# Maxwell-Zhao/RoboSimGS

Hardware: AMD Instinct MI355X
Metric: frames/sec + ms/frame (fwd, fwd+bwd) at 1M Gaussians 1920x1080 (higher is better)
Workload: dtype f32

## Files before the change

### include/mgs.h

```cpp
#ifndef MGS_H_
#define MGS_H_

#include <stddef.h>
#include <stdint.h>

#ifdef __cplusplus
extern "C" {
#endif

#define MGS_VERSION 450

#define MGS_OK 0
#define MGS_ERR_INVALID_ARGUMENT (-1)
#define MGS_ERR_WORKSPACE_TOO_SMALL (-2)
#define MGS_ERR_UNSUPPORTED (-3)

#define MGS_STATUS_ISECT_OVERFLOW 1u

#define MGS_RASTER_EXPECTED_LAST 1
#define MGS_RASTER_LATENCY 2

#define MGS_FRAMES_CLASSIC_BOUNDS 4

#define MGS_FRAMES_RADIUS_OPACITY_AWARE 8
#define MGS_FRAMES_CAMERA_ORTHO 16
#define MGS_FRAMES_CAMERA_FISHEYE 32

#define MGS_CAMERA_PINHOLE 0
#define MGS_CAMERA_ORTHO 1
#define MGS_CAMERA_FISHEYE 2

#ifndef MGS_RADIUS_CLASSIC
#define MGS_RADIUS_CLASSIC 0
#define MGS_RADIUS_OPACITY_AWARE 1
#endif
#define MGS_BIN_TIGHT 1
#define MGS_BIN_RADIUS_OPACITY_AWARE 2
#define MGS_BIN_CAMERA_ORTHO 4
#define MGS_BIN_CAMERA_FISHEYE 8

#define MGS_PARAMS_RAW 64
#define MGS_PARAMS_OPAC_PLAIN 128

#define MGS_RASTER_BWD_SPLAT_SLOTS 2
#define MGS_RASTER_BWD_RECORDS_ONLY 1

#define MGS_TILE_SIZE 16
#define MGS_MAX_CHANNELS 32

typedef void *mgs_stream_t;

int mgs_version(void);
const char *mgs_last_error_string(void);
#ifdef MGS_DEBUG_HOOKS
void mgs_debug_set_raster_cull(int enabled);
void mgs_debug_set_raster_opts(int opts);
void mgs_debug_set_sort_opts(int opts);
#endif

int mgs_projection_fwd(int n, const float *means, const float *quats, const float *scales,
                       const float *viewmat, const float *K, int width, int height,
                       float eps2d, float near_plane, float far_plane, float radius_clip,
                       int32_t *radii, float *means2d, float *depths, float *conics,
                       float *compensations, const float *opacities, int radius_rule,
                       int32_t *radii_y, int camera_model, mgs_stream_t stream);

int mgs_projection_bwd(int n, const float *means, const float *quats, const float *scales,
                       const float *viewmat, const float *K, int width, int height,
                       float eps2d, const int32_t *radii, const float *conics,
                       const float *compensations, const float *v_means2d,
                       const float *v_depths, const float *v_conics,
                       const float *v_compensations, float *v_means, float *v_quats,
                       float *v_scales, float *v_viewmat, int camera_model, mgs_stream_t stream);

int mgs_sh_fwd(int n, int degree, int coeff_stride, const float *dirs, const float *coeffs,
               const uint8_t *masks, float *colors, mgs_stream_t stream);
int mgs_sh_bwd(int n, int degree, int coeff_stride, const float *dirs, const float *coeffs,
               const uint8_t *masks, const float *v_colors, float *v_coeffs, float *v_dirs,
               mgs_stream_t stream);

int mgs_project_color_fwd(int n, const float *means, const float *quats, const float *scales,
                          const float *opacities, int sh_degree, int coeff_stride,
                          const float *sh_coeffs, const float *viewmat, const float *K,
                          int width, int height, float eps2d, float near_plane,
                          float far_plane, float radius_clip, int32_t *radii, float *means2d,
                          float *depths, float *conics, float *opac_out, int feat_stride,
                          float *feats, float *splats, int bin_flags, uint32_t *bin_info,
                          uint32_t *bin_sums, int32_t *radii_y, mgs_stream_t stream);

int mgs_isect_tiles(int n, const float *means2d, const int32_t *radii, const int32_t *radii_y, const float *depths,
                    const float *conics, const float *opacities, int tile_size, int tile_w,
                    int tile_h, int cam_id, int n_cams,
                    uint32_t isect_capacity, int32_t *tiles_per_gauss, uint32_t *n_isect,
                    uint32_t *tile_ids, int32_t *flatten_ids, int64_t *isect_ids,
                    int32_t *tile_offsets, int32_t *pair_info, int32_t *tile_group_order,
                    uint32_t *status, const uint32_t *seed_info, uint32_t *seed_sums, float *splat_slots,
                    void *workspace, size_t *workspace_bytes, mgs_stream_t stream);

int mgs_render_frames(int n, const float *means, const float *quats, const float *scales,
                      const float *opacities, int sh_degree, int coeff_stride, const float *sh_coeffs,
                      int n_cams, const float *viewmats, const float *Ks, int width, int height,
                      float eps2d, float near_plane, float far_plane, float radius_clip,
                      int antialiased, int channels, int flags, const float *backgrounds,
                      uint32_t isect_capacity, float *render, float *alphas, uint32_t *n_isect,
                      uint32_t *status, uint8_t *ds_rgba, void *ds_distance, int ds_distance_type,
                      const double *ds_Kinv_host, void *workspace, size_t *workspace_bytes, mgs_stream_t stream);

#define MGS_TRAIN_FIELDS 17
int mgs_train_state_layout(int n, int width, int height, int channels, uint32_t isect_capacity, int antialiased,
                           int checkpoint_interval, size_t *offsets, size_t *bytes_per_camera);
int mgs_render_frames_train(int n, const float *means, const float *quats, const float *scales,
                            const float *opacities, int sh_degree, int coeff_stride, const float *sh_coeffs,
                            int n_cams, const float *viewmats, const float *Ks, int width, int height,
                            float eps2d, float near_plane, float far_plane, float radius_clip, int antialiased,
                            int channels, int flags, const float *backgrounds, uint32_t isect_capacity,
                            int checkpoint_interval, float *render, float *alphas, void *state, void *workspace,
                            size_t *workspace_bytes, mgs_stream_t stream);
int mgs_render_frames_backward(int n, const float *means, const float *quats, const float *scales,
                               const float *opacities, int sh_degree, int coeff_stride, const float *sh_coeffs,
                               int n_cams, const float *viewmats, const float *Ks, int width, int height,
                               float eps2d, int antialiased, int channels, int flags, const float *backgrounds,
                               uint32_t isect_capacity, int checkpoint_interval, const float *render,
                               const float *alphas, const float *v_render, const float *v_alphas,
                               const void *state, float *v_means, float *v_quats, float *v_scales,
                               float *v_sh_coeffs, float *v_opacities, float *v_viewmats, float *v_means2d,
                               float *v_means2d_abs, void *workspace, size_t *workspace_bytes,
                               mgs_stream_t stream);

int mgs_isect_offset_encode(uint32_t n_isect, const int64_t *isect_ids, int n_cams,
                            int tile_w, int tile_h, int32_t *offsets, mgs_stream_t stream);

int mgs_rasterize_fwd(int n, const float *means2d, const float *conics, const float *feats,
                      const float *opacities, const float *splats, const float *background,
                      int channels, int width, int height, int tile_w, int tile_h,
                      const int32_t *tile_offsets, const int32_t *flatten_ids,
                      const int32_t *tile_group_order, int flags,
                      float *render, float *alphas, int32_t *last_ids, float *checkpoints,
                      int checkpoint_interval, uint8_t *ds_rgba, void *ds_distance, int ds_distance_type,
                      const double *ds_Kinv_host, mgs_stream_t stream);
size_t mgs_raster_checkpoint_floats(uint32_t isect_capacity, int tile_w, int tile_h, int channels,
                                    int checkpoint_interval);

int mgs_rasterize_bwd(int n, const float *means2d, const float *conics, const float *feats,
                      const float *opacities, const float *background, int channels,
                      int width, int height, int tile_w, int tile_h,
                      const int32_t *tile_offsets, const int32_t *flatten_ids,
                      const float *alphas, const int32_t *last_ids, const float *v_render,
                      const float *v_alphas, float *v_means2d, float *v_means2d_abs,
                      float *v_conics, float *v_feats, float *v_opacities,
                      mgs_stream_t stream);

int mgs_rasterize_bwd_det(int n, const float *means2d, const float *conics, const float *feats,
                          const float *opacities, const float *splats, const float *background,
                          int channels, int width, int height, int tile_w, int tile_h,
                          const int32_t *tile_offsets, const int32_t *flatten_ids,
                          const float *alphas, const int32_t *last_ids, const float *v_render,
                          const float *v_alphas, const float *expected_render,
                          const int32_t *pair_info, const int32_t *tile_group_order,
                          uint32_t isect_capacity, const float *render_out, const float *checkpoints,
                          int checkpoint_interval, int flags, float *v_means2d, float *v_means2d_abs,
                          float *v_conics, float *v_feats, float *v_opacities, void *workspace,
                          size_t *workspace_bytes, mgs_stream_t stream);

int mgs_project_color_bwd(int n, const float *means, const float *quats, const float *scales,
                          const float *opacities, int sh_degree, int coeff_stride,
                          const float *sh_coeffs, const float *viewmat, const float *K,
                          int width, int height, float eps2d, const int32_t *radii,
                          const float *conics, int antialiased, int feat_stride,
                          const float *feats, const float *v_feats, const float *v_means2d,
                          const float *v_conics, const float *v_depths,
                          const float *v_opac_out, float *v_means, float *v_quats,
                          float *v_scales, float *v_sh_coeffs, float *v_opacities,
                          float *v_viewmat, int accumulate, int camera_model, mgs_stream_t stream);

int mgs_composite_over(int n_px, const float *bg_rgb, const float *bg_alpha,
                       const float *bg_depth, const float *fg_rgb, const float *fg_depth,
                       const uint8_t *fg_mask, const float *backdrop, float *out_rgb,
                       float *out_depth, mgs_stream_t stream);

int mgs_frame_to_u8(int n_px, const float *rgb, int rgb_stride, const float *alpha,
                    const float *background, uint8_t *out, mgs_stream_t stream);

int mgs_frame_to_dataset(int width, int height, const float *colors, int color_stride,
                         const float *alpha, const float *background, const double *Kinv_host,
                         uint8_t *rgba, void *distance, int distance_f64, mgs_stream_t stream);

int mgs_points_project(int n, const float *pts, const float *K, const float *c2w, float *uv,
                       float *pnt_cam, mgs_stream_t stream);
int mgs_points_depth_map(int n, const float *uv, int uv_stride, const float *depth, int height,
                         int width, int cells_h, int cells_w, float scale, float bg_depth,
                         float *depth_map, int64_t *index, void *workspace,
                         size_t *workspace_bytes, mgs_stream_t stream);
int mgs_points_sample_mask(int n, const float *uv, int uv_stride, const float *mask, int height,
                           int width, float thresh, const float *depth_map,
                           const float *pnt_depth, float depth_thresh, uint8_t *out,
                           mgs_stream_t stream);

#define MGS_SSIM_VALID 0
#define MGS_SSIM_SAME 1

typedef struct mgs_image_loss {
  int images, height, width, channels;
  float ssim_weight;
  int padding;
} mgs_image_loss;

int mgs_l1_loss_fwd(size_t n, const float *a, const float *b, float *loss, void *workspace,
                    size_t *workspace_bytes, mgs_stream_t stream, const mgs_image_loss *image);
int mgs_l1_loss_bwd(size_t n, const float *a, const float *b, const float *v_loss, float *v_a,
                    mgs_stream_t stream, const mgs_image_loss *image);
int mgs_l1_loss_fwd_grad(size_t n, const float *a, const float *b, float *loss, float *v_a,
                         void *workspace, size_t *workspace_bytes, mgs_stream_t stream,
                         const mgs_image_loss *image);
int mgs_l1_loss_bwd_scale(size_t n, const float *v_loss, float *v_a, mgs_stream_t stream);

int mgs_transform_gaussians(int n, const float *means, const float *quats, const float *scales,
                            int sh_degree, int coeff_stride, const float *sh_coeffs,
                            const int32_t *group_ids, int n_groups, const float *xforms,
                            const float *sh_rot, float *out_means, float *out_quats,
                            float *out_scales, float *out_sh, mgs_stream_t stream);

#ifdef __cplusplus
}
#endif
#endif
```

### robosimgs_amd/csrc/binning.hip

```cpp
#include "mgs_common.h"
#include "tile_rect.h"
#include "tile_order.h"

namespace mgs {
namespace {

constexpr int kBlock = 128;

__device__ __forceinline__ uint32_t wave_sum(uint32_t v) {
#pragma unroll
  for (int d = 32; d >= 1; d >>= 1) v += __shfl_xor(v, d);
  return v;
}

constexpr int kSum = 64;
__global__ __launch_bounds__(kBlock) void tile_count_kernel(
    int n, const float* __restrict__ means2d, const int32_t* __restrict__ radii,
    const int32_t* __restrict__ radii_y, const float* __restrict__ conics, const float* __restrict__ opacities,
    float tile_size, int tile_w, int tile_h, uint2* __restrict__ ginfo, uint32_t* __restrict__ sums) {
  int g = blockIdx.x * kBlock + threadIdx.x;
  int radius = g < n ? radii[g] : 0;
  uint2 info = make_uint2(kEmptyTileRect, 0u);
  if (radius > 0) {
    float2 m = reinterpret_cast<const float2*>(means2d)[g];
    TileRect r = tile_rect(m.x, m.y, radius, radii_y ? radii_y[g] : radius, tile_size, tile_w, tile_h);
    if (conics)
      r = tighten_rect(r, m.x, m.y, conics[3 * (size_t)g], conics[3 * (size_t)g + 1],
                       conics[3 * (size_t)g + 2], opacities[g], tile_size);
    info = pack_tile_rect(r);
  }
  if (g < n) ginfo[g] = info;
  const uint32_t c = wave_sum(info.y);
  const int first = blockIdx.x * kBlock + (int)(threadIdx.x & ~63u);
  if ((threadIdx.x & 63) == 0 && first < n) sums[first / kSum] = c;
}

constexpr int kScanThreads = 1024;
constexpr int kScanPerThread = 16;
template <int kScanThreads>
__device__ __forceinline__ void scan_blocksums_body(
    uint32_t nblk, uint32_t* __restrict__ blocksums, uint32_t capacity,
    uint32_t* __restrict__ n_isect, uint32_t* __restrict__ status) {
  __shared__ uint32_t ws[kScanThreads / 64];
  const unsigned lane = threadIdx.x & 63, wave = threadIdx.x >> 6;
  uint32_t running = 0;
  bool wrapped = false;
  for (uint32_t b0 = 0; b0 < nblk; b0 += kScanThreads * kScanPerThread) {
    const uint32_t b = b0 + threadIdx.x * kScanPerThread;
    uint32_t v[kScanPerThread], sum = 0;
    if (b + kScanPerThread <= nblk) {
      const uint4* src = reinterpret_cast<const uint4*>(blocksums + b);
      const uint4 q0 = src[0], q1 = src[1], q2 = src[2], q3 = src[3];
      v[0] = q0.x; v[1] = q0.y; v[2] = q0.z; v[3] = q0.w; v[4] = q1.x; v[5] = q1.y; v[6] = q1.z; v[7] = q1.w;
      v[8] = q2.x; v[9] = q2.y; v[10] = q2.z; v[11] = q2.w; v[12] = q3.x; v[13] = q3.y; v[14] = q3.z; v[15] = q3.w;
    } else {
#pragma unroll
      for (int j = 0; j < kScanPerThread; ++j) v[j] = b + j < nblk ? blocksums[b + j] : 0u;
    }
#pragma unroll
    for (int j = 0; j < kScanPerThread; ++j) sum += v[j];
    uint32_t incl = sum;
#pragma unroll
    for (int d = 1; d < 64; d <<= 1) {
      uint32_t t = __shfl_up(incl, d);
      if (lane >= (unsigned)d) incl += t;
    }
    if (lane == 63) ws[wave] = incl;
    __syncthreads();
    uint32_t off = 0, tot = 0;
    for (int w = 0; w < kScanThreads / 64; ++w) {
      if ((unsigned)w < wave) off += ws[w];
      tot += ws[w];
    }
    __syncthreads();
    uint32_t ex = running + off + incl - sum;
    uint32_t o[kScanPerThread];
#pragma unroll
    for (int j = 0; j < kScanPerThread; ++j) { o[j] = ex; ex += v[j]; }
    if (b + kScanPerThread <= nblk) {
      uint4* dst = reinterpret_cast<uint4*>(blocksums + b);
      dst[0] = make_uint4(o[0], o[1], o[2], o[3]);
      dst[1] = make_uint4(o[4], o[5], o[6], o[7]);
      dst[2] = make_uint4(o[8], o[9], o[10], o[11]);
      dst[3] = make_uint4(o[12], o[13], o[14], o[15]);
    } else {
#pragma unroll
      for (int j = 0; j < kScanPerThread; ++j)
        if (b + j < nblk) blocksums[b + j] = o[j];
    }
    wrapped |= running + tot < running;
    running += tot;
  }
  if (threadIdx.x == 0 && n_isect) {
    *n_isect = wrapped ? 0xffffffffu : running;
    *status = (wrapped || running > capacity) ? MGS_STATUS_ISECT_OVERFLOW : 0u;
  }
}
__global__ __launch_bounds__(kScanThreads) void scan_blocksums_kernel(
    uint32_t nblk, uint32_t* __restrict__ blocksums, uint32_t capacity,
    uint32_t* __restrict__ n_isect, uint32_t* __restrict__ status) {
  scan_blocksums_body<kScanThreads>(nblk, blocksums, capacity, n_isect, status);
}

__device__ __forceinline__ void store_splat_slots(float* __restrict__ splat_slots, int g, uint32_t slot_base, uint32_t rect) {
  if (splat_slots)
    *reinterpret_cast<uint2*>(splat_slots + 12 * (size_t)g + 10) = make_uint2(slot_base, rect & 0x3fffffffu);
}

__global__ __launch_bounds__(kBlock) void pair_info_kernel(
    int n, const uint2* __restrict__ ginfo, int tile_h, const uint32_t* __restrict__ blockbase,
    int4* __restrict__ pair_info, float* __restrict__ splat_slots) {
  __shared__ uint32_t ws[kBlock / 64];
  const unsigned lane = threadIdx.x & 63, wave = threadIdx.x >> 6;
  int g = blockIdx.x * kBlock + threadIdx.x;
  uint2 info = g < n ? ginfo[g] : make_uint2(1u << 20, 0u);
  uint32_t cnt = info.y;
  uint32_t incl = cnt;
#pragma unroll
  for (int d = 1; d < 64; d <<= 1) {
    uint32_t t = __shfl_up(incl, d);
    if (lane >= (unsigned)d) incl += t;
  }
  if (lane == 63) ws[wave] = incl;
  __syncthreads();
  uint32_t off = 0;
  for (int w = 0; w < kBlock / 64; ++w)
    if ((unsigned)w < wave) off += ws[w];
  if (g < n) {
    const uint32_t w = info.x >> 20;
    const uint32_t slot_base = blockbase[blockIdx.x * (kBlock / kSum)] + off + incl - cnt;
    pair_info[g] = cnt ? make_int4((int)slot_base, (int)(info.x & 1023u),
                                   (int)((info.x >> 10) & 1023u), (int)(w | ((cnt / w) << 16)))
                       : make_int4(0, 0, 0, 0);
    if (cnt) store_splat_slots(splat_slots, g, slot_base, info.x);
  }
}

__global__ __launch_bounds__(kBlock) void emit_kernel(
    int n, const uint2* __restrict__ ginfo, int tile_w, const uint32_t* __restrict__ blockbase,
    uint32_t capacity, uint32_t* __restrict__ tile_out, uint32_t* __restrict__ id_out,
    int32_t* __restrict__ tiles_per_gauss) {
  __shared__ uint32_t prefix[kBlock + 1];
  __shared__ uint32_t gid[kBlock];
  __shared__ uint32_t rpack[kBlock];
  __shared__ uint32_t ws[kBlock / 64];
  const unsigned lane = threadIdx.x & 63, wave = threadIdx.x >> 6;
  int r = blockIdx.x * kBlock + threadIdx.x;
  uint32_t cnt = 0, g = (uint32_t)r, pack = 1u << 20;
  if (r < n) {
    uint2 info = ginfo[r];
    pack = info.x;
    cnt = info.y;
    if (tiles_per_gauss) tiles_per_gauss[r] = (int32_t)cnt;
  }
  uint32_t incl = cnt;
#pragma unroll
  for (int d = 1; d < 64; d <<= 1) {
    uint32_t t = __shfl_up(incl, d);
    if (lane >= (unsigned)d) incl += t;
  }
  if (lane == 63) ws[wave] = incl;
  __syncthreads();
  uint32_t off = 0, total = 0;
  for (int w = 0; w < kBlock / 64; ++w) {
    if ((unsigned)w < wave) off += ws[w];
    total += ws[w];
  }
  prefix[threadIdx.x] = off + incl - cnt;
  if (threadIdx.x == 0) prefix[kBlock] = total;
  gid[threadIdx.x] = g;
  rpack[threadIdx.x] = pack;
  __syncthreads();
  const uint32_t base = blockbase[blockIdx.x * (kBlock / kSum)];
  for (uint32_t k0 = threadIdx.x * 4u; k0 < total; k0 += kBlock * 4u) {
    int lo = 0, hi = kBlock;
    while (hi - lo > 1) {
      int mid = (lo + hi) >> 1;
      if (prefix[mid] <= k0) lo = mid; else hi = mid;
    }
    uint32_t next = prefix[lo + 1];
    uint32_t tiles4[4], ids4[4];
#pragma unroll
    for (int i = 0; i < 4; ++i) {
      uint32_t k = k0 + i;
      while (k >= next && lo < kBlock - 1) next = prefix[++lo + 1];
      uint32_t local = k - prefix[lo];
      uint32_t p = rpack[lo];
      uint32_t w = p >> 20;
      uint32_t dy = local / w;
      uint32_t dx = local - dy * w;
      tiles4[i] = (((p >> 10) & 1023u) + dy) * (uint32_t)tile_w + (p & 1023u) + dx;
      ids4[i] = gid[lo];
    }
#pragma unroll
    for (int i = 0; i < 4; ++i) {
      uint32_t out = base + k0 + i;
      if (k0 + i < total && out < capacity) {
        tile_out[out] = tiles4[i];
        id_out[out] = ids4[i];
      }
    }
  }
}


constexpr int kDirectThreads = 512;
constexpr int kDealRun = 256;
static_assert(kDealRun % 64 == 0 && kDirectThreads % kDealRun == 0 && kDirectThreads >= kDealRun,
              "kDirectThreads must be a multiple of kDealRun, and the run a multiple of the wave");
constexpr int kDirectPerThread = 4;
constexpr int kDirectMaxBlocks = 1024;
constexpr int kDirectMaxTiles = 15000;
constexpr int kGroupShift = 2;
constexpr uint32_t kCoopRect = 24;
constexpr uint32_t kRunRect = 128;

template <class F>
__device__ __forceinline__ void for_each_tile(uint32_t pack, uint32_t cnt, uint32_t g, int tile_w, F f) {
  const bool big = cnt > kCoopRect;
  if (!big) {
    const uint32_t w = pack >> 20;
    uint32_t t = ((pack >> 10) & 1023u) * (uint32_t)tile_w + (pack & 1023u), dx = 0;
    for (uint32_t k = 0; k < cnt; ++k) {
      f(t + dx, g);
      if (++dx == w) { dx = 0; t += (uint32_t)tile_w; }
    }
  }
  unsigned long long m = ballot(big);
  const unsigned lane = lane_id();
  while (m) {
    const int src = __ffsll((long long)m) - 1;
    m &= m - 1;
    const uint32_t p = __shfl(pack, src), c = __shfl(cnt, src), gs = __shfl(g, src);
    const uint32_t w = p >> 20, x0 = p & 1023u, y0 = (p >> 10) & 1023u;
    for (uint32_t k = lane; k < c; k += 64) {
      const uint32_t dy = k / w, dx = k - dy * w;
      f((y0 + dy) * (uint32_t)tile_w + x0 + dx, gs);
    }
  }
}

template <class F>
__device__ __forceinline__ void for_each_tile_run(uint32_t pack, uint32_t cnt, uint32_t g, int tile_w, int shift, F f) {
  const bool big = cnt > kCoopRect;
  if (!big) {
    const uint32_t w = pack >> 20;
    uint32_t t = ((pack >> 10) & 1023u) * (uint32_t)tile_w + (pack & 1023u), dx = 0;
    for (uint32_t k = 0; k < cnt; ++k) {
      f(t + dx, 1u, g);
      if (++dx == w) { dx = 0; t += (uint32_t)tile_w; }
    }
  }
  unsigned long long m = ballot(big);
  const unsigned lane = lane_id();
  const uint32_t G = 1u << shift;
  while (m) {
    const int src = __ffsll((long long)m) - 1;
    m &= m - 1;
    const uint32_t p = __shfl(pack, src), c = __shfl(cnt, src), gs = __shfl(g, src);
    const uint32_t w = p >> 20, x0 = p & 1023u, y0 = (p >> 10) & 1023u, h = c / w;
    const uint32_t R = (w + G - 2u) / G + 1u;
    const int lr = R > 1u ? 32 - __clz((int)(R - 1u)) : 0;
    if (lr > 6 || c <= kRunRect) {
      for (uint32_t k = lane; k < c; k += 64) {
        const uint32_t dy = k / w, dx = k - dy * w;
        f((y0 + dy) * (uint32_t)tile_w + x0 + dx, 1u, gs);
      }
      continue;
    }
    const uint32_t rows_per_trip = 64u >> lr, r = lane >> lr, j = lane & ((1u << lr) - 1u);
    for (uint32_t dy0 = 0; dy0 < h; dy0 += rows_per_trip) {
      const uint32_t dy = dy0 + r;
      const uint32_t t0 = (y0 + dy) * (uint32_t)tile_w + x0, bin = (t0 >> shift) + j;
      const uint32_t lo = max(t0, bin << shift), hi = min(t0 + w, (bin + 1u) << shift);
      if (dy < h && lo < hi) f(lo, hi - lo, gs);
    }
  }
}

struct DealtIndex {
  int g0, g1, n, deal_nb;
  __device__ __forceinline__ int operator()(int base, int i) const {
    if (deal_nb > 0) {
      const int pass = (base - g0) / (kDirectThreads * kDirectPerThread);
      constexpr int R = kDealRun, kSub = kDirectThreads / R;
      const int sub = (int)threadIdx.x / R, within = (int)threadIdx.x % R;
      const long long g = (((long long)(pass * kDirectPerThread + i) * kSub + sub) * deal_nb + blockIdx.x) * R + within;
      return g < n ? (int)g : -1;
    }
    const int g = base + i * kDirectThreads + (int)threadIdx.x;
    return g < g1 ? g : -1;
  }
};

__global__ __launch_bounds__(kDirectThreads) void direct_hist_kernel(
    int n, int chunk, const uint2* __restrict__ ginfo, int tile_w, int n_tiles, int shift,
    uint32_t* __restrict__ table, int32_t* __restrict__ tiles_per_gauss, uint32_t* __restrict__ scan_sums, uint32_t n_sums,
    int deal_nb) {
  extern __shared__ uint32_t hist[];
  if (scan_sums && blockIdx.x == gridDim.x - 1) {
    scan_blocksums_body<kDirectThreads>(n_sums, scan_sums, 0u, nullptr, nullptr);
    return;
  }
  n_tiles = (n_tiles + (1 << shift) - 1) >> shift;
  for (int i = threadIdx.x; i < n_tiles; i += kDirectThreads) hist[i] = 0u;
  __syncthreads();
  const int g0 = blockIdx.x * chunk, g1 = min(n, g0 + chunk);
  const DealtIndex gi{g0, g1, n, deal_nb};
  const int g_end = deal_nb > 0 ? g0 + chunk : g1;
  for (int base = g0; base < g_end; base += kDirectThreads * kDirectPerThread) {
    uint2 info[kDirectPerThread];
#pragma unroll
    for (int i = 0; i < kDirectPerThread; ++i) {
      const int g = gi(base, i);
      info[i] = g >= 0 ? ginfo[g] : make_uint2(kEmptyTileRect, 0u);
    }
#pragma unroll
    for (int i = 0; i < kDirectPerThread; ++i) {
      const int g = gi(base, i);
      if (g >= 0 && tiles_per_gauss) tiles_per_gauss[g] = (int32_t)info[i].y;
      if (shift > 0)
        for_each_tile_run(info[i].x, info[i].y, (uint32_t)g, tile_w, shift, [&](uint32_t tile, uint32_t n_run, uint32_t) { atomicAdd(&hist[tile >> shift], n_run); });
      else
        for_each_tile(info[i].x, info[i].y, (uint32_t)g, tile_w, [&](uint32_t tile, uint32_t) { atomicAdd(&hist[tile >> shift], 1u); });
    }
  }
  __syncthreads();
  uint32_t* row = table + (size_t)blockIdx.x * n_tiles;
  for (int i = threadIdx.x; i < n_tiles; i += kDirectThreads) row[i] = hist[i];
}

constexpr int kColThreads = 256, kColBins = 16, kColGroups = kColThreads / kColBins, kColKeepTraining = 32;
template <int kColKeep>
__global__ __launch_bounds__(kColThreads) void direct_colscan_kernel(
    int nb, int n_tiles, uint32_t* __restrict__ table, uint32_t* __restrict__ tile_count) {
  __shared__ uint32_t part[kColGroups][kColBins];
  const int bl = threadIdx.x % kColBins, rg = threadIdx.x / kColBins;
  const int t = blockIdx.x * kColBins + bl;
  const int rpg = (nb + kColGroups - 1) / kColGroups;
  const int r0 = rg * rpg, r1 = min(nb, r0 + rpg);
  const bool ok = t < n_tiles;
  constexpr bool kCanKeep = kColKeep > 1;
  const bool keep = kCanKeep && rpg <= kColKeep;
  uint32_t kept[kColKeep];
  uint32_t sum = 0;
  if (kCanKeep && keep) {
#pragma unroll
    for (int j = 0; j < kColKeep; ++j) {
      if (j >= rpg) { kept[j] = 0u; continue; }
      kept[j] = (ok && r0 + j < r1) ? table[(size_t)(r0 + j) * n_tiles + t] : 0u;
    }
#pragma unroll
    for (int j = 0; j < kColKeep; ++j) sum += kept[j];
  } else {
    for (int r = r0; r < r1; r += 16) {
      uint32_t v[16];
#pragma unroll
      for (int j = 0; j < 16; ++j) v[j] = (ok && r + j < r1) ? table[(size_t)(r + j) * n_tiles + t] : 0u;
#pragma unroll
      for (int j = 0; j < 16; ++j) sum += v[j];
    }
  }
  part[rg][bl] = sum;
  __syncthreads();
  uint32_t off = 0, tot = 0;
#pragma unroll 16
  for (int g = 0; g < kColGroups; ++g) {
    const uint32_t s = part[g][bl];
    if (g < rg) off += s;
    tot += s;
  }
  if (kCanKeep && keep) {
#pragma unroll
    for (int j = 0; j < kColKeep; ++j) {
      if (j >= rpg) continue;
      if (ok && r0 + j < r1) {
        table[(size_t)(r0 + j) * n_tiles + t] = off;
        off += kept[j];
      }
    }
  } else {
    for (int r = r0; r < r1; r += 16) {
      uint32_t v[16];
#pragma unroll
      for (int j = 0; j < 16; ++j) v[j] = (ok && r + j < r1) ? table[(size_t)(r + j) * n_tiles + t] : 0u;
#pragma unroll
      for (int j = 0; j < 16; ++j)
        if (ok && r + j < r1) {
          table[(size_t)(r + j) * n_tiles + t] = off;
          off += v[j];
        }
    }
  }
  if (rg == 0 && ok) tile_count[t] = tot;
}

template <bool PAIRS>
__global__ __launch_bounds__(kDirectThreads) void direct_scatter_kernel(
    int n, int chunk, const uint2* __restrict__ ginfo, int tile_w, int n_tiles, int shift,
    const uint32_t* __restrict__ table, const uint32_t* __restrict__ tile_count, uint32_t capacity,
    uint32_t* __restrict__ flatten_ids, int32_t* __restrict__ tile_offsets,
    uint32_t* __restrict__ n_isect, uint32_t* __restrict__ status, int32_t* __restrict__ group_order,
    const uint32_t* __restrict__ scanned_sums, int4* __restrict__ pair_info, uint32_t* __restrict__ zero_word,
    float* __restrict__ splat_slots, int deal_nb) {
  extern __shared__ uint32_t cursor[];
  n_tiles = (n_tiles + (1 << shift) - 1) >> shift;
  if (group_order && blockIdx.x == gridDim.x - 1) {
    order_groups_by_total<kDirectThreads>(n_tiles, [&](int g) { return tile_count[g]; }, group_order);
    return;
  }
  const uint32_t local_mask = (1u << shift) - 1u;
  __shared__ unsigned long long wsum[kDirectThreads / 64];
  const unsigned lane = threadIdx.x & 63, wave = threadIdx.x >> 6;
  const int per = (n_tiles + kDirectThreads - 1) / kDirectThreads;
  const int t0 = (int)threadIdx.x * per;
  unsigned long long sum = 0;
  for (int k = 0; k < per; ++k)
    if (t0 + k < n_tiles) sum += tile_count[t0 + k];
  unsigned long long incl = sum;
#pragma unroll
  for (int d = 1; d < 64; d <<= 1) {
    const uint32_t lo = __shfl_up((uint32_t)incl, d), hi = __shfl_up((uint32_t)(incl >> 32), d);
    if (lane >= (unsigned)d) incl += ((unsigned long long)hi << 32) | lo;
  }
  if (lane == 63) wsum[wave] = incl;
  __syncthreads();
  unsigned long long off = 0, total = 0;
#pragma unroll
  for (int w = 0; w < kDirectThreads / 64; ++w) {
    if ((unsigned)w < wave) off += wsum[w];
    total += wsum[w];
  }
  unsigned long long ex = off + incl - sum;
  const uint32_t* row = table + (size_t)blockIdx.x * n_tiles;
  for (int k = 0; k < per; ++k) {
    const int t = t0 + k;
    if (t < n_tiles) {
      const uint32_t at = ex < capacity ? (uint32_t)ex : capacity;
      cursor[t] = ex < capacity ? at + row[t] : capacity;
      if (blockIdx.x == 0) tile_offsets[t] = (int32_t)at;
      ex += tile_count[t];
    }
  }
  if (blockIdx.x == 0 && threadIdx.x == 0) {
    tile_offsets[n_tiles] = (int32_t)(total < capacity ? (uint32_t)total : capacity);
    *n_isect = total > 0xffffffffull ? 0xffffffffu : (uint32_t)total;
    *status = total > capacity ? MGS_STATUS_ISECT_OVERFLOW : 0u;
    if (zero_word) reinterpret_cast<uint4*>(zero_word)[0] = reinterpret_cast<uint4*>(zero_word)[1] = make_uint4(0u, 0u, 0u, 0u);
  }
  __syncthreads();
  const int g0 = blockIdx.x * chunk, g1 = min(n, g0 + chunk);
  const DealtIndex gi{g0, g1, n, deal_nb};
  const int g_end = deal_nb > 0 ? g0 + chunk : g1;
  for (int base = g0; base < g_end; base += kDirectThreads * kDirectPerThread) {
    uint2 info[kDirectPerThread];
#pragma unroll
    for (int i = 0; i < kDirectPerThread; ++i) {
      const int g = gi(base, i);
      info[i] = g >= 0 ? ginfo[g] : make_uint2(kEmptyTileRect, 0u);
    }
    if (PAIRS) {
      uint32_t sbase[kDirectPerThread];
#pragma unroll
      for (int i = 0; i < kDirectPerThread; ++i) {
        const int g = gi(base, i);
        sbase[i] = g >= 0 ? scanned_sums[g / kSum] : 0u;
      }
#pragma unroll
      for (int i = 0; i < kDirectPerThread; ++i) {
        const int g = gi(base, i);
        const uint32_t cnt = info[i].y;
        uint32_t incl = cnt;
#pragma unroll
        for (int d = 1; d < 64; d <<= 1) {
          const uint32_t t = __shfl_up(incl, d);
          if (lane >= (unsigned)d) incl += t;
        }
        if (g >= 0) {
          const uint32_t w = info[i].x >> 20;
          pair_info[g] = cnt ? make_int4((int)(sbase[i] + incl - cnt), (int)(info[i].x & 1023u), (int)((info[i].x >> 10) & 1023u),
                                         (int)(w | ((cnt / w) << 16)))
                             : make_int4(0, 0, 0, 0);
          if (cnt) store_splat_slots(splat_slots, g, sbase[i] + incl - cnt, info[i].x);
        }
      }
    }
#pragma unroll
    for (int i = 0; i < kDirectPerThread; ++i) {
      const int g = gi(base, i);
      if (shift > 0)
        for_each_tile_run(info[i].x, info[i].y, (uint32_t)g, tile_w, shift, [&](uint32_t tile, uint32_t n_run, uint32_t gs) {
          const uint32_t p = atomicAdd(&cursor[tile >> shift], n_run);
          for (uint32_t k = 0; k < n_run; ++k)
            if (p + k < capacity) flatten_ids[p + k] = gs | (((tile + k) & local_mask) << (32 - shift));
        });
      else
      for_each_tile(info[i].x, info[i].y, (uint32_t)g, tile_w, [&](uint32_t tile, uint32_t gs) {
        const uint32_t p = atomicAdd(&cursor[tile >> shift], 1u);
        if (p < capacity) flatten_ids[p] = shift ? gs | ((tile & local_mask) << (32 - shift)) : gs;
      });
    }
  }
}

constexpr int kOffsetsPerThread = 8;
__global__ __launch_bounds__(kBlock) void tile_offsets_kernel(
    const uint32_t* __restrict__ n_ptr, uint32_t capacity, const uint32_t* __restrict__ tiles,
    int n_tiles, int32_t* __restrict__ offsets) {
  uint32_t n = min(*n_ptr, capacity);
  uint32_t t = blockIdx.x * kBlock + threadIdx.x;
  if (n == 0) {
    for (uint32_t k = t; k <= (uint32_t)n_tiles; k += gridDim.x * kBlock) offsets[k] = 0;
    return;
  }
  uint32_t i0 = t * kOffsetsPerThread;
  if (i0 >= n) return;
  uint32_t v[kOffsetsPerThread];
  if (i0 + kOffsetsPerThread <= n) {
    const uint4 a = *reinterpret_cast<const uint4*>(tiles + i0), b = *reinterpret_cast<const uint4*>(tiles + i0 + 4);
    v[0] = a.x; v[1] = a.y; v[2] = a.z; v[3] = a.w; v[4] = b.x; v[5] = b.y; v[6] = b.z; v[7] = b.w;
  } else {
#pragma unroll
    for (int j = 0; j < kOffsetsPerThread; ++j) v[j] = i0 + j < n ? tiles[i0 + j] : 0u;
  }
  int prev = i0 ? (int)tiles[i0 - 1] : -1;
#pragma unroll
  for (int j = 0; j < kOffsetsPerThread; ++j) {
    const uint32_t i = i0 + j;
    if (i < n) {
      const int cur = (int)v[j];
      for (int k = prev + 1; k <= cur; ++k) offsets[k] = (int32_t)i;
      prev = cur;
      if (i == n - 1)
        for (int k = cur + 1; k <= n_tiles; ++k) offsets[k] = (int32_t)n;
    }
  }
}

__global__ __launch_bounds__(kBlock) void isect_ids_kernel(
    const uint32_t* __restrict__ n_ptr, uint32_t capacity, const uint32_t* __restrict__ tiles,
    const int32_t* __restrict__ ids, const float* __restrict__ depths, int64_t cam_shifted,
    int64_t* __restrict__ isect_ids) {
  uint32_t n = min(*n_ptr, capacity);
  uint32_t i = blockIdx.x * kBlock + threadIdx.x;
  if (i >= n) return;
  int64_t hi = cam_shifted | (int64_t)tiles[i];
  isect_ids[i] = (hi << 32) | (int64_t)__float_as_uint(depths[ids[i]]);
}

__global__ __launch_bounds__(kBlock) void offset_encode_kernel(
    uint32_t n, const int64_t* __restrict__ isect_ids, int n_cams, int n_tiles, int tile_bits,
    int32_t* __restrict__ offsets) {
  uint32_t i = blockIdx.x * kBlock + threadIdx.x;
  int total = n_cams * n_tiles;
  if (n == 0) {
    for (uint32_t k = i; k < (uint32_t)total; k += gridDim.x * kBlock) offsets[k] = 0;
    return;
  }
  if (i >= n) return;
  auto flat = [&](int64_t key) {
    int64_t t = key >> 32;
    return (int)((t >> tile_bits) * n_tiles + (t & ((1ll << tile_bits) - 1)));
  };
  int cur = flat(isect_ids[i]);
  int prev = i ? flat(isect_ids[i - 1]) : -1;
  for (int k = prev + 1; k <= cur && k < total; ++k) offsets[k] = (int32_t)i;
  if (i == n - 1)
    for (int k = cur + 1; k < total; ++k) offsets[k] = (int32_t)n;
}

__global__ __launch_bounds__(1024) void tile_group_order_kernel(int n_tiles, const int32_t* __restrict__ tile_offsets,
                                                                int32_t* __restrict__ order) {
  order_groups_by_total<1024>((n_tiles + 3) / 4, [&](int g) {
    return (uint32_t)(tile_offsets[min(4 * g + 4, n_tiles)] - tile_offsets[4 * g]);
  }, order);
}

int bits_for(uint32_t count) {
  int b = 0;
  while (count > 1 && (1ull << b) < count) ++b;
  return b;
}

unsigned direct_chunk(unsigned n) {
  const unsigned per_block = max(div_up(n, kDirectMaxBlocks), (unsigned)(kDirectThreads * kDirectPerThread));
  return div_up(per_block, kDirectThreads) * kDirectThreads;
}
unsigned direct_blocks(unsigned n) { return div_up(n, direct_chunk(n)); }

struct Workspace {
  size_t total;
  size_t ginfo, blocksums, tile_alt, tile_priv, id_alt, radix, tsort, table, tile_count, group_offsets;
  Workspace(int n, uint32_t cap, int n_tiles) {
    Bump b(0);
    size_t nn = (size_t)(n > 0 ? n : 1), cc = cap ? cap : 1;
    ginfo = b.take(nn * 8);
    blocksums = b.take((size_t)div_up((unsigned)nn, kSum) * 4);
    tile_alt = b.take(cc * 4); id_alt = b.take(cc * 4);
    tile_priv = b.take(cc * 4);
    radix = b.take(radix_sort_temp_bytes((uint32_t)cc));
    tsort = b.take(tile_depth_sort_temp_bytes((uint32_t)cc, n_tiles));
    const size_t nt = (size_t)(n_tiles < kDirectMaxTiles ? n_tiles : kDirectMaxTiles);
    table = b.take((size_t)direct_blocks((unsigned)nn) * nt * 4);
    tile_count = b.take(nt * 4);
    group_offsets = b.take((nt + 1) * 4);
    total = b.total;
  }
};

}
}

namespace mgs {
size_t isect_tiles_workspace_bytes(int n, uint32_t capacity, int n_tiles) { return Workspace(n, capacity, n_tiles).total; }

int launch_tile_group_order(int n_tiles, const int32_t* tile_offsets, int32_t* order, hipStream_t stream) {
  hipLaunchKernelGGL(tile_group_order_kernel, dim3(1), dim3(1024), 0, stream, n_tiles, tile_offsets, order);
  return check_launch("tile_group_order");
}
}

using namespace mgs;

extern "C" int mgs_isect_tiles(int n, const float* means2d, const int32_t* radii, const int32_t* radii_y,
                               const float* depths, const float* conics, const float* opacities,
                               int tile_size, int tile_w, int tile_h,
                               int cam_id, int n_cams, uint32_t isect_capacity,
                               int32_t* tiles_per_gauss, uint32_t* n_isect, uint32_t* tile_ids,
                               int32_t* flatten_ids, int64_t* isect_ids, int32_t* tile_offsets,
                               int32_t* pair_info, int32_t* tile_group_order, uint32_t* status,
                               const uint32_t* seed_info,
                               uint32_t* seed_sums, float* splat_slots, void* workspace,
                               size_t* workspace_bytes, mgs_stream_t stream) {
  MGS_REQUIRE(n >= 0 && tile_size > 0 && tile_w > 0 && tile_h > 0, "isect_tiles: bad sizes");
  MGS_REQUIRE(tile_w <= 1023 && tile_h <= 1023, "isect_tiles: tile grid %dx%d exceeds 1023x1023", tile_w, tile_h);
  MGS_REQUIRE(workspace_bytes, "isect_tiles: workspace_bytes is null");
  MGS_REQUIRE(cam_id >= 0 && n_cams > cam_id, "isect_tiles: cam_id %d outside 0..%d", cam_id, n_cams);
  const Workspace ws(n, isect_capacity, tile_w * tile_h);
  if (!workspace) {
    *workspace_bytes = ws.total;
    return MGS_OK;
  }
  if (*workspace_bytes < ws.total)
    return set_error(MGS_ERR_WORKSPACE_TOO_SMALL, "isect_tiles: workspace %zu < %zu bytes",
                     *workspace_bytes, ws.total);
  MGS_REQUIRE(isect_capacity > 0, "isect_tiles: zero capacity");
  MGS_REQUIRE(seed_info || (conics == nullptr) == (opacities == nullptr),
              "isect_tiles: tight tile bounds need both conics and opacities");
  MGS_REQUIRE(n == 0 || (seed_info == nullptr) == (seed_sums == nullptr),
              "isect_tiles: seed_info and seed_sums come together (mgs_project_color_fwd writes both)");
  MGS_REQUIRE((n == 0 || ((seed_info || (means2d && radii)) && depths)) && n_isect && flatten_ids &&
                  tile_offsets && status, "isect_tiles: null pointer");
  MGS_REQUIRE(!seed_info || tile_size == MGS_TILE_SIZE, "isect_tiles: a seed is for tile_size %d, got %d", MGS_TILE_SIZE, tile_size);
  MGS_REQUIRE(!seed_sums || (reinterpret_cast<uintptr_t>(seed_sums) & 15u) == 0, "isect_tiles: seed_sums must be 16-byte aligned");
  MGS_REQUIRE(!splat_slots || pair_info, "isect_tiles: splat_slots are written with pair_info");
  MGS_REQUIRE(!splat_slots || (reinterpret_cast<uintptr_t>(splat_slots) & 15u) == 0, "isect_tiles: splat_slots must be 16-byte aligned");
  hipStream_t s = (hipStream_t)stream;
  char* w = static_cast<char*>(workspace);
  auto u32 = [&](size_t off) { return reinterpret_cast<uint32_t*>(w + off); };
  const bool want_tile_ids = tile_ids != nullptr;
  if (!tile_ids) tile_ids = u32(ws.tile_priv);
  const int n_tiles = tile_w * tile_h;
  const uint32_t cap = isect_capacity;
  const int gshift = (sort_opts() & 8) ? (sort_opts() >> 4) & 7 : kGroupShift;
  const bool direct = ((n_tiles + (1 << gshift) - 1) >> gshift) <= kDirectMaxTiles && !(sort_opts() & 4) &&
                      (gshift == 0 || (unsigned)n <= (1u << (32 - gshift)));
  int rc;
  bool order_done = false;

  if (n == 0) {
    (void)hipMemsetAsync(n_isect, 0, 4, s);
    (void)hipMemsetAsync(status, 0, 4, s);
  } else {
    const unsigned nblk = div_up(n, kBlock), nsum = div_up(n, kSum);
    const uint2* ginfo = reinterpret_cast<const uint2*>(seed_info);
    uint32_t* sums = seed_sums;
    if (!seed_info) {
      uint2* gi = reinterpret_cast<uint2*>(w + ws.ginfo);
      sums = u32(ws.blocksums);
      hipLaunchKernelGGL(tile_count_kernel, dim3(nblk), dim3(kBlock), 0, s, n, means2d, radii, radii_y, conics,
                         opacities, (float)tile_size, tile_w, tile_h, gi, sums);
      ginfo = gi;
    }
    if (direct) {
      const int chunk = (int)direct_chunk((unsigned)n);
      const unsigned nb = direct_blocks((unsigned)n);
      const int bins = (n_tiles + (1 << gshift) - 1) >> gshift;
      const size_t lds = (size_t)bins * sizeof(uint32_t);
      const int deal_nb = (int)nb;
      hipLaunchKernelGGL(direct_hist_kernel, dim3(nb + (pair_info ? 1 : 0)), dim3(kDirectThreads), lds, s, n, chunk, ginfo, tile_w,
                         n_tiles, gshift, u32(ws.table), tiles_per_gauss, pair_info ? sums : nullptr, nsum, deal_nb);
      if (pair_info)
        hipLaunchKernelGGL(direct_colscan_kernel<kColKeepTraining>, dim3(div_up((unsigned)bins, (unsigned)kColBins)), dim3(kColThreads), 0, s,
                           (int)nb, bins, u32(ws.table), u32(ws.tile_count));
      else
        hipLaunchKernelGGL(direct_colscan_kernel<1>, dim3(div_up((unsigned)bins, (unsigned)kColBins)), dim3(kColThreads), 0, s,
                           (int)nb, bins, u32(ws.table), u32(ws.tile_count));
      const bool order_in_scatter = tile_group_order && gshift == 2;
      order_done = order_in_scatter;
      with_bool(pair_info != nullptr, [&](auto training) {
        hipLaunchKernelGGL(direct_scatter_kernel<decltype(training)::value>, dim3(nb + (order_in_scatter ? 1 : 0)),
                           dim3(kDirectThreads), lds, s, n, chunk, ginfo, tile_w, n_tiles, gshift, u32(ws.table),
                           u32(ws.tile_count), cap, gshift ? u32(ws.id_alt) : reinterpret_cast<uint32_t*>(flatten_ids),
                           gshift ? reinterpret_cast<int32_t*>(w + ws.group_offsets) : tile_offsets, n_isect, status,
                           order_in_scatter ? tile_group_order : nullptr, sums, reinterpret_cast<int4*>(pair_info),
                           tile_depth_sort_long_list(w + ws.tsort, cap), pair_info ? splat_slots : nullptr, deal_nb);
      });
    } else {
      hipLaunchKernelGGL(scan_blocksums_kernel, dim3(1), dim3(kScanThreads), 0, s, nsum, sums, cap,
                         n_isect, status);
      const int tile_bits = bits_for((uint32_t)n_tiles);
      const int passes = (tile_bits + 7) / 8;
      uint32_t* user_t = tile_ids;
      uint32_t* user_i = reinterpret_cast<uint32_t*>(flatten_ids);
      uint32_t *a_t = user_t, *a_i = user_i, *b_t = u32(ws.tile_alt), *b_i = u32(ws.id_alt);
      if (passes & 1) { a_t = u32(ws.tile_alt); a_i = u32(ws.id_alt); b_t = user_t; b_i = user_i; }
      hipLaunchKernelGGL(emit_kernel, dim3(nblk), dim3(kBlock), 0, s, n, ginfo, tile_w, sums, cap, a_t,
                         a_i, tiles_per_gauss);
      if (pair_info)
        hipLaunchKernelGGL(pair_info_kernel, dim3(nblk), dim3(kBlock), 0, s, n, ginfo, tile_h, sums,
                           reinterpret_cast<int4*>(pair_info), splat_slots);
      rc = radix_sort_pairs(n_isect, cap, tile_bits, a_t, a_i, b_t, b_i, w + ws.radix, s);
      if (rc) return rc;
    }
  }
  if (!direct || n == 0)
    hipLaunchKernelGGL(tile_offsets_kernel, dim3(div_up(cap, kBlock * kOffsetsPerThread)), dim3(kBlock), 0,
                       s, n_isect, cap, tile_ids, n_tiles, tile_offsets);
  if (n > 0) {
    const bool grouped = direct && gshift > 0;
    rc = tile_depth_sort(n_tiles, tile_offsets, depths, cap, reinterpret_cast<uint32_t*>(flatten_ids),
                         direct && (want_tile_ids || isect_ids) ? tile_ids : nullptr, w + ws.tsort, s,
                          u32(ws.tile_alt), u32(ws.id_alt),
                         grouped ? u32(ws.id_alt) : nullptr,
                         grouped ? reinterpret_cast<const int32_t*>(w + ws.group_offsets) : nullptr, gshift, direct);
    if (rc) return rc;
  }
  if (tile_group_order && !order_done) {
    rc = launch_tile_group_order(n_tiles, tile_offsets, tile_group_order, s);
    if (rc) return rc;
  }
  const unsigned gblk = div_up(cap, kBlock);
  if (isect_ids) {
    const int tile_bits_key = bits_for((uint32_t)n_tiles + 1);
    hipLaunchKernelGGL(isect_ids_kernel, dim3(gblk), dim3(kBlock), 0, s, n_isect, cap, tile_ids,
                       flatten_ids, depths, (int64_t)cam_id << tile_bits_key, isect_ids);
  }
  return check_launch("isect_tiles");
}

extern "C" int mgs_isect_offset_encode(uint32_t n_isect, const int64_t* isect_ids, int n_cams,
                                       int tile_w, int tile_h, int32_t* offsets,
                                       mgs_stream_t stream) {
  MGS_REQUIRE(n_cams > 0 && tile_w > 0 && tile_h > 0, "isect_offset_encode: bad sizes");
  MGS_REQUIRE(offsets && (isect_ids || n_isect == 0), "isect_offset_encode: null pointer");
  const int n_tiles = tile_w * tile_h;
  const int tile_bits = bits_for((uint32_t)n_tiles + 1);
  unsigned gblk = n_isect ? div_up(n_isect, kBlock) : div_up((unsigned)(n_cams * n_tiles), kBlock);
  hipLaunchKernelGGL(offset_encode_kernel, dim3(gblk), dim3(kBlock), 0, (hipStream_t)stream,
                     n_isect, isect_ids, n_cams, n_tiles, tile_bits, offsets);
  return check_launch("isect_offset_encode");
}
```

### robosimgs_amd/csrc/build.py

```python
from __future__ import annotations

import hashlib
import os
import shutil
import subprocess
import sys
from concurrent.futures import ThreadPoolExecutor

HERE = os.path.dirname(os.path.abspath(__file__))
SOURCES = ["api.hip", "projection.hip", "sort.hip", "binning.hip", "tile_sort.hip", "raster_fwd.hip",
           "raster_bwd.hip", "backward.hip", "composite.hip", "points.hip", "loss.hip", "transform.hip", "frame.hip",
           "optim.hip", "refine.hip"]
HEADERS = ["mgs_common.h", "mgs_math.h", "raster_common.h", "sh_staging.h", "tile_rect.h", "tile_order.h",
           "../../include/mgs.h", "../../include/mgs_optim.h",
           "../../include/mgs_refine.h"]
LIB = os.path.join(HERE, "libmgs.so")
DEBUG_LIB = os.path.join(HERE, "libmgs_debug.so")
HOOK_SOURCES = ["raster_fwd.hip", "sort.hip"]
OBJ_DIR = os.path.join(HERE, "build")
FLAGS = ["--offload-arch=gfx950", "-O3", "-std=c++17", "-fPIC", "-munsafe-fp-atomics",
         "-fno-slp-vectorize", "-Wall", "-Wno-unused-function"] + os.environ.get("MGS_EXTRA_FLAGS", "").split()


PER_SOURCE_FLAGS = {
    "raster_bwd.hip": os.environ.get("MGS_RASTER_BWD_FLAGS", "").split(),
    "raster_fwd.hip": os.environ.get("MGS_RASTER_FWD_FLAGS", "").split(),
    "tile_sort.hip": os.environ.get("MGS_TILE_SORT_FLAGS", "").split(),
    "binning.hip": os.environ.get("MGS_BINNING_FLAGS", "").split(),
}


def _hipcc() -> str:
    for c in (os.environ.get("HIPCC"), shutil.which("hipcc"), "/opt/rocm/bin/hipcc"):
        if c and os.path.exists(c):
            return c
    raise RuntimeError("hipcc not found; libmgs.so cannot be built")


def _stamp() -> str:
    h = hashlib.sha256((" ".join(FLAGS) + repr(sorted(PER_SOURCE_FLAGS.items()))).encode())
    for f in SOURCES + HEADERS:
        p = os.path.join(HERE, f)
        if os.path.exists(p):
            with open(p, "rb") as fh:
                h.update(fh.read())
    return h.hexdigest()


def _code_only(text: str) -> str:
    out, i, n = [], 0, len(text)
    while i < n:
        c = text[i]
        if c in "\"'":
            j = i + 1
            while j < n and text[j] != c:
                j += 2 if text[j] == "\\" else 1
            out.append(text[i:j + 1])
            i = j + 1
        elif text.startswith("//", i):
            j = text.find("\n", i)
            i = n if j < 0 else j
        elif text.startswith("/*", i):
            j = text.find("*/", i + 2)
            i = n if j < 0 else j + 2
            out.append(" ")
        else:
            out.append(c)
            i += 1
    return " ".join("".join(out).split())


def current_stamp() -> str:
    h = hashlib.sha256((" ".join(FLAGS) + repr(sorted(PER_SOURCE_FLAGS.items()))).encode())
    for f in SOURCES + HEADERS:
        p = os.path.join(HERE, f)
        if os.path.exists(p):
            with open(p, "r", encoding="utf-8", errors="replace") as fh:
                h.update(_code_only(fh.read()).encode())
    return h.hexdigest()


def build(force: bool = False, verbose: bool = False) -> str:
    stamp_file = os.path.join(OBJ_DIR, "stamp")
    stamp = _stamp()
    if (not force and os.path.exists(LIB) and os.path.exists(DEBUG_LIB) and os.path.exists(stamp_file)
            and open(stamp_file).read() == stamp):
        return LIB
    os.makedirs(OBJ_DIR, exist_ok=True)
    hipcc = _hipcc()
    srcs = [s for s in SOURCES if os.path.exists(os.path.join(HERE, s))]

    def compile_one(job) -> str:
        src, hooks = job
        obj = os.path.join(OBJ_DIR, src.replace(".hip", ".dbg.o" if hooks else ".o"))
        cmd = [hipcc, *FLAGS, *PER_SOURCE_FLAGS.get(src, []), *(["-DMGS_DEBUG_HOOKS"] if hooks else []), "-c",
               os.path.join(HERE, src), "-o", obj]
        if verbose:
            print(" ".join(cmd), flush=True)
        r = subprocess.run(cmd, capture_output=True, text=True)
        if r.returncode != 0:
            raise RuntimeError(f"hipcc failed on {src}:\n{r.stderr}")
        if verbose and r.stderr.strip():
            print(r.stderr, file=sys.stderr)
        return obj

    jobs = [(s_, False) for s_ in srcs] + [(s_, True) for s_ in srcs if s_ in HOOK_SOURCES]
    with ThreadPoolExecutor(max_workers=4) as ex:
        objs = dict(zip(jobs, ex.map(compile_one, jobs)))
    for lib, hooks in ((LIB, False), (DEBUG_LIB, True)):
        use = [objs[(s_, hooks and s_ in HOOK_SOURCES)] for s_ in srcs]
        cmd = [hipcc, "--offload-arch=gfx950", "-shared", "-fPIC", *use, "-o", lib]
        r = subprocess.run(cmd, capture_output=True, text=True)
        if r.returncode != 0:
            raise RuntimeError(f"link failed:\n{r.stderr}")
    with open(stamp_file, "w") as f:
        f.write(stamp)
    return LIB


if __name__ == "__main__":
    print(build(force="--force" in sys.argv, verbose=True))
```

### robosimgs_amd/csrc/frame.hip

```cpp
#include "mgs_common.h"

namespace {
struct Frames {
  int tile_w, tile_h, n_tiles;
  int bin_flags;
  int camera_model;
  bool raw;
};
int frames_prologue(const char* fn, int n, int n_cams, int width, int height, int channels, int flags, const float* opacities,
                    uint32_t isect_capacity, const size_t* workspace_bytes, Frames* f,
                    const char* channel_rule = "3 (RGB) or 4 (RGB + depth)") {
  MGS_REQUIRE(n >= 0 && n_cams >= 1 && width > 0 && height > 0, "%s: bad sizes", fn);
  MGS_REQUIRE(channels == 3 || channels == 4, "%s: channels must be %s, got %d", fn, channel_rule, channels);
  MGS_REQUIRE(workspace_bytes, "%s: workspace_bytes is null", fn);
  MGS_REQUIRE(isect_capacity > 0, "%s: zero capacity", fn);
  MGS_REQUIRE((flags & (MGS_FRAMES_CAMERA_ORTHO | MGS_FRAMES_CAMERA_FISHEYE)) != (MGS_FRAMES_CAMERA_ORTHO | MGS_FRAMES_CAMERA_FISHEYE),
              "%s: flags set both MGS_FRAMES_CAMERA_ORTHO and MGS_FRAMES_CAMERA_FISHEYE", fn);
  f->raw = (flags & MGS_PARAMS_RAW) != 0;
  MGS_REQUIRE(!f->raw || opacities, "%s: MGS_PARAMS_RAW needs opacities (the logits), got NULL", fn);
  f->tile_w = (width + MGS_TILE_SIZE - 1) / MGS_TILE_SIZE;
  f->tile_h = (height + MGS_TILE_SIZE - 1) / MGS_TILE_SIZE;
  f->n_tiles = f->tile_w * f->tile_h;
  f->bin_flags = ((flags & MGS_FRAMES_CLASSIC_BOUNDS) ? 0 : MGS_BIN_TIGHT ) |
                 ((flags & MGS_FRAMES_RADIUS_OPACITY_AWARE) ? MGS_BIN_RADIUS_OPACITY_AWARE : 0) |
                 ((flags & MGS_FRAMES_CAMERA_ORTHO) ? MGS_BIN_CAMERA_ORTHO : 0) |
                 ((flags & MGS_FRAMES_CAMERA_FISHEYE) ? MGS_BIN_CAMERA_FISHEYE : 0) | (f->raw ? MGS_PARAMS_RAW : 0);
  f->camera_model = mgs::bin_camera_model(f->bin_flags);
  return MGS_OK;
}
int isect_bytes(int n, uint32_t isect_capacity, const Frames& f, size_t* bytes) {
  MGS_REQUIRE(f.tile_w <= 1023 && f.tile_h <= 1023, "isect_tiles: tile grid %dx%d exceeds 1023x1023", f.tile_w, f.tile_h);
  *bytes = mgs::isect_tiles_workspace_bytes(n, isect_capacity, f.n_tiles);
  return MGS_OK;
}

struct FrameWs {
  size_t total, depths, opac, splats, bin_info, bin_sums, flatten, offsets, order, isect;
  size_t isect_bytes;
  FrameWs(int n, uint32_t cap, int n_tiles, bool antialiased, size_t isect_ws) {
    mgs::Bump b(1);
    const size_t nn = (size_t)(n > 0 ? n : 1);
    depths = b.take(nn * 4);
    opac = b.take(antialiased ? nn * 4 : 0);
    splats = b.take(nn * 48);
    bin_info = b.take(nn * 8);
    bin_sums = b.take(((nn + 63) / 64) * 4);
    flatten = b.take((size_t)cap * 4);
    offsets = b.take(((size_t)n_tiles + 1) * 4);
    order = b.take((((size_t)n_tiles + 3) / 4) * 4);
    isect = b.take(isect_ws);
    isect_bytes = isect_ws;
    total = b.total;
  }
};
}

extern "C" int mgs_render_frames(int n, const float* means, const float* quats, const float* scales,
                                 const float* opacities, int sh_degree, int coeff_stride, const float* sh_coeffs,
                                 int n_cams, const float* viewmats, const float* Ks, int width, int height,
                                 float eps2d, float near_plane, float far_plane, float radius_clip,
                                 int antialiased, int channels, int flags, const float* backgrounds,
                                 uint32_t isect_capacity, float* render, float* alphas, uint32_t* n_isect,
                                 uint32_t* status, uint8_t* ds_rgba, void* ds_distance, int ds_distance_type,
                                 const double* ds_Kinv_host, void* workspace, size_t* workspace_bytes, mgs_stream_t stream) {
  Frames f;
  int rc = frames_prologue("render_frames", n, n_cams, width, height, channels, flags, opacities, isect_capacity, workspace_bytes, &f);
  if (rc) return rc;
  if ((ds_rgba || ds_distance) && f.camera_model != MGS_CAMERA_PINHOLE)
    return mgs::set_error(MGS_ERR_UNSUPPORTED, "render_frames: dataset output (ds_rgba / ds_distance) converts depth to ray "
                                               "distance through a pinhole K^-1; it is not available for an orthographic "
                                               "or fisheye camera");
  const int tile_w = f.tile_w, tile_h = f.tile_h;
  size_t isect_ws = 0;
  rc = isect_bytes(n, isect_capacity, f, &isect_ws);
  if (rc) return rc;
  const FrameWs ws(n, isect_capacity, f.n_tiles, antialiased != 0, isect_ws);
  if (!workspace) {
    *workspace_bytes = ws.total;
    return MGS_OK;
  }
  if (*workspace_bytes < ws.total)
    return mgs::set_error(MGS_ERR_WORKSPACE_TOO_SMALL, "render_frames: workspace %zu < %zu bytes", *workspace_bytes, ws.total);
  MGS_REQUIRE(viewmats && Ks && ((render && alphas) || (ds_rgba && !render && !alphas)) && n_isect && status,
              "render_frames: null pointer");
  MGS_REQUIRE(ds_distance_type >= 0 && ds_distance_type <= 2, "render_frames: distance type %d not in {0: f32, 1: f64, 2: f16}",
              ds_distance_type);
  const size_t ds_dist_bytes = ds_distance_type == 1 ? 8 : (ds_distance_type == 2 ? 2 : 4);
  MGS_REQUIRE((reinterpret_cast<uintptr_t>(workspace) & 255u) == 0, "render_frames: workspace must be 256-byte aligned");
  char* w = static_cast<char*>(workspace);
  float* depths = reinterpret_cast<float*>(w + ws.depths);
  float* opac_aa = antialiased ? reinterpret_cast<float*>(w + ws.opac) : nullptr;
  float* splats = reinterpret_cast<float*>(w + ws.splats);
  uint32_t* bin_info = reinterpret_cast<uint32_t*>(w + ws.bin_info);
  uint32_t* bin_sums = reinterpret_cast<uint32_t*>(w + ws.bin_sums);
  int32_t* flatten = reinterpret_cast<int32_t*>(w + ws.flatten);
  int32_t* offsets = reinterpret_cast<int32_t*>(w + ws.offsets);
  int32_t* order = reinterpret_cast<int32_t*>(w + ws.order);
  const size_t n_px = (size_t)width * height;
  for (int c = 0; c < n_cams; ++c) {
    rc = mgs_project_color_fwd(n, means, quats, scales, opacities, sh_degree, coeff_stride, sh_coeffs,
                               viewmats + 16 * (size_t)c, Ks + 9 * (size_t)c, width, height, eps2d, near_plane, far_plane,
                               radius_clip, nullptr, nullptr, depths, nullptr, opac_aa, channels, nullptr, splats, f.bin_flags,
                               bin_info, bin_sums, nullptr, stream);
    if (rc) return rc;
    size_t iw = ws.isect_bytes;
    rc = mgs_isect_tiles(n, nullptr, nullptr, nullptr, depths, nullptr, nullptr, MGS_TILE_SIZE, tile_w, tile_h, 0, 1,
                         isect_capacity, nullptr, n_isect + c, nullptr, flatten, nullptr, offsets, nullptr, order,
                         status + c, bin_info, bin_sums, nullptr, w + ws.isect, &iw, stream);
    if (rc) return rc;
    rc = mgs_rasterize_fwd(n, nullptr, nullptr, nullptr, nullptr, splats, backgrounds ? backgrounds + (size_t)channels * c : nullptr,
                           channels, width, height, tile_w, tile_h, offsets, flatten, order,
                           flags & (MGS_RASTER_EXPECTED_LAST | MGS_RASTER_LATENCY),
                           render ? render + n_px * channels * c : nullptr, alphas ? alphas + n_px * c : nullptr, nullptr, nullptr, 0,
                           ds_rgba ? ds_rgba + n_px * 4 * c : nullptr,
                           ds_distance ? static_cast<char*>(ds_distance) + n_px * ds_dist_bytes * c : nullptr, ds_distance_type,
                           ds_Kinv_host, stream);
    if (rc) return rc;
  }
  return MGS_OK;
}

namespace {
enum TrainField { TF_RADII, TF_MEANS2D, TF_DEPTHS, TF_CONICS, TF_OPAC, TF_FEATS, TF_SPLATS, TF_TILES_PER_GAUSS, TF_PAIR_INFO,
                  TF_TILE_IDS, TF_FLATTEN, TF_OFFSETS, TF_ORDER, TF_LAST_IDS, TF_CKPT, TF_COUNTS, TF_RADII_Y, TF_FIELDS };
static_assert(TF_FIELDS == MGS_TRAIN_FIELDS, "mgs.h: MGS_TRAIN_FIELDS");
struct TrainState {
  size_t at[TF_FIELDS], total;
  TrainState(int n, int width, int height, int channels, uint32_t cap, bool antialiased, int interval) {
    const int tile_w = (width + MGS_TILE_SIZE - 1) / MGS_TILE_SIZE, tile_h = (height + MGS_TILE_SIZE - 1) / MGS_TILE_SIZE;
    const size_t nn = (size_t)(n > 0 ? n : 1), n_tiles = (size_t)tile_w * tile_h, n_px = (size_t)width * height;
    mgs::Bump b(1);
    auto take = [&](int f, size_t bytes) { at[f] = b.take(bytes); };
    take(TF_RADII, nn * 4);
    take(TF_MEANS2D, nn * 8);
    take(TF_DEPTHS, nn * 4);
    take(TF_CONICS, nn * 12);
    take(TF_OPAC, antialiased ? nn * 4 : 0);
    take(TF_FEATS, nn * 4 * channels);
    take(TF_SPLATS, nn * 48);
    take(TF_TILES_PER_GAUSS, nn * 4);
    take(TF_PAIR_INFO, nn * 16);
    take(TF_TILE_IDS, (size_t)cap * 4);
    take(TF_FLATTEN, (size_t)cap * 4);
    take(TF_OFFSETS, (n_tiles + 1) * 4);
    take(TF_ORDER, ((n_tiles + 3) / 4) * 4);
    take(TF_LAST_IDS, n_px * 4);
    take(TF_CKPT, interval ? mgs_raster_checkpoint_floats(cap, tile_w, tile_h, channels, interval) * 4 : 0);
    take(TF_COUNTS, 8);
    take(TF_RADII_Y, nn * 4);
    total = b.total;
  }
};
struct TrainWs {
  size_t bin_info, bin_sums, isect, total;
  TrainWs(int n, size_t isect_ws) {
    mgs::Bump b(1);
    const size_t nn = (size_t)(n > 0 ? n : 1);
    bin_info = b.take(nn * 8);
    bin_sums = b.take(((nn + 63) / 64) * 4);
    isect = b.take(isect_ws);
    total = b.total;
  }
};
struct BwdWs {
  size_t v_means2d, v_abs, v_conics, v_feats, v_opac, raster, total;
  BwdWs(int n, int channels, size_t raster_ws) {
    mgs::Bump b(1);
    const size_t nn = (size_t)(n > 0 ? n : 1);
    v_means2d = b.take(nn * 8);
    v_abs = b.take(nn * 8);
    v_conics = b.take(nn * 12);
    v_feats = b.take(nn * 4 * channels);
    v_opac = b.take(nn * 4);
    raster = b.take(raster_ws);
    total = b.total;
  }
};
__global__ __launch_bounds__(256) void add_rows_kernel(size_t n, const float* __restrict__ src, float* __restrict__ dst, int first) {
  const size_t i = (size_t)blockIdx.x * 256 + threadIdx.x;
  if (i < n) dst[i] = first ? src[i] : dst[i] + src[i];
}
}

extern "C" int mgs_train_state_layout(int n, int width, int height, int channels, uint32_t isect_capacity, int antialiased,
                                      int checkpoint_interval, size_t* offsets, size_t* bytes_per_camera) {
  MGS_REQUIRE(n >= 0 && width > 0 && height > 0 && (channels == 3 || channels == 4) && isect_capacity > 0 && bytes_per_camera,
              "train_state_layout: bad arguments");
  MGS_REQUIRE(checkpoint_interval == 0 || (checkpoint_interval >= 64 && (checkpoint_interval & (checkpoint_interval - 1)) == 0),
              "train_state_layout: checkpoint_interval %d is not 0 or a power of two >= 64", checkpoint_interval);
  const TrainState st(n, width, height, channels, isect_capacity, antialiased != 0, checkpoint_interval);
  if (offsets)
    for (int f = 0; f < TF_FIELDS; ++f) offsets[f] = st.at[f];
  *bytes_per_camera = st.total;
  return MGS_OK;
}

extern "C" int mgs_render_frames_train(int n, const float* means, const float* quats, const float* scales,
                                       const float* opacities, int sh_degree, int coeff_stride, const float* sh_coeffs,
                                       int n_cams, const float* viewmats, const float* Ks, int width, int height,
                                       float eps2d, float near_plane, float far_plane, float radius_clip, int antialiased,
                                       int channels, int flags, const float* backgrounds, uint32_t isect_capacity,
                                       int checkpoint_interval, float* render, float* alphas, void* state, void* workspace,
                                       size_t* workspace_bytes, mgs_stream_t stream) {
  Frames f;
  int rc = frames_prologue("render_frames_train", n, n_cams, width, height, channels, flags, opacities, isect_capacity, workspace_bytes,
                           &f);
  if (rc) return rc;
  const int tile_w = f.tile_w, tile_h = f.tile_h;
  size_t isect_ws = 0;
  rc = isect_bytes(n, isect_capacity, f, &isect_ws);
  if (rc) return rc;
  const TrainWs ws(n, isect_ws);
  if (!workspace) {
    *workspace_bytes = ws.total;
    return MGS_OK;
  }
  if (*workspace_bytes < ws.total)
    return mgs::set_error(MGS_ERR_WORKSPACE_TOO_SMALL, "render_frames_train: workspace %zu < %zu bytes", *workspace_bytes, ws.total);
  MGS_REQUIRE(viewmats && Ks && render && alphas && state, "render_frames_train: null pointer");
  MGS_REQUIRE(((reinterpret_cast<uintptr_t>(workspace) | reinterpret_cast<uintptr_t>(state)) & 255u) == 0,
              "render_frames_train: workspace and state must be 256-byte aligned");
  MGS_REQUIRE(checkpoint_interval == 0 || (checkpoint_interval >= 64 && (checkpoint_interval & (checkpoint_interval - 1)) == 0),
              "render_frames_train: checkpoint_interval %d is not 0 or a power of two >= 64", checkpoint_interval);
  const bool keep_opac = antialiased != 0 || f.raw;
  const TrainState st(n, width, height, channels, isect_capacity, keep_opac, checkpoint_interval);
  const int bin_flags = f.bin_flags | ((f.raw && !antialiased) ? MGS_PARAMS_OPAC_PLAIN : 0);
  char* w = static_cast<char*>(workspace);
  uint32_t* bin_info = reinterpret_cast<uint32_t*>(w + ws.bin_info);
  uint32_t* bin_sums = reinterpret_cast<uint32_t*>(w + ws.bin_sums);
  const size_t n_px = (size_t)width * height;
  for (int c = 0; c < n_cams; ++c) {
    char* s = static_cast<char*>(state) + st.total * (size_t)c;
    auto F = [&](int f) { return reinterpret_cast<float*>(s + st.at[f]); };
    auto I = [&](int f) { return reinterpret_cast<int32_t*>(s + st.at[f]); };
    auto U = [&](int f) { return reinterpret_cast<uint32_t*>(s + st.at[f]); };
    float* opac_aa = keep_opac ? F(TF_OPAC) : nullptr;
    rc = mgs_project_color_fwd(n, means, quats, scales, opacities, sh_degree, coeff_stride, sh_coeffs,
                               viewmats + 16 * (size_t)c, Ks + 9 * (size_t)c, width, height, eps2d, near_plane, far_plane,
                               radius_clip, I(TF_RADII), F(TF_MEANS2D), F(TF_DEPTHS), F(TF_CONICS), opac_aa, channels,
                               F(TF_FEATS), F(TF_SPLATS), bin_flags, bin_info, bin_sums, I(TF_RADII_Y), stream);
    if (rc) return rc;
    size_t iw = isect_ws;
    rc = mgs_isect_tiles(n, nullptr, nullptr, nullptr, F(TF_DEPTHS), nullptr, nullptr, MGS_TILE_SIZE, tile_w, tile_h, c, n_cams,
                         isect_capacity, I(TF_TILES_PER_GAUSS), U(TF_COUNTS), U(TF_TILE_IDS), I(TF_FLATTEN), nullptr,
                         I(TF_OFFSETS), I(TF_PAIR_INFO), I(TF_ORDER), U(TF_COUNTS) + 1, bin_info, bin_sums, F(TF_SPLATS),
                         w + ws.isect, &iw, stream);
    if (rc) return rc;
    rc = mgs_rasterize_fwd(n, nullptr, nullptr, nullptr, nullptr, F(TF_SPLATS),
                           backgrounds ? backgrounds + (size_t)channels * c : nullptr, channels, width, height, tile_w, tile_h,
                           I(TF_OFFSETS), I(TF_FLATTEN), I(TF_ORDER), flags & (MGS_RASTER_EXPECTED_LAST | MGS_RASTER_LATENCY),
                           render + n_px * channels * c, alphas + n_px * c, I(TF_LAST_IDS),
                           checkpoint_interval ? F(TF_CKPT) : nullptr, checkpoint_interval, nullptr, nullptr, 0, nullptr, stream);
    if (rc) return rc;
  }
  return MGS_OK;
}

extern "C" int mgs_render_frames_backward(int n, const float* means, const float* quats, const float* scales,
                                          const float* opacities, int sh_degree, int coeff_stride, const float* sh_coeffs,
                                          int n_cams, const float* viewmats, const float* Ks, int width, int height,
                                          float eps2d, int antialiased, int channels, int flags, const float* backgrounds,
                                          uint32_t isect_capacity, int checkpoint_interval, const float* render,
                                          const float* alphas, const float* v_render, const float* v_alphas,
                                          const void* state, float* v_means, float* v_quats, float* v_scales,
                                          float* v_sh_coeffs, float* v_opacities, float* v_viewmats, float* v_means2d,
                                          float* v_means2d_abs, void* workspace, size_t* workspace_bytes,
                                          mgs_stream_t stream) {
  Frames f;
  int rc = frames_prologue("render_frames_backward", n, n_cams, width, height, channels, flags, opacities, isect_capacity,
                           workspace_bytes, &f, "3 or 4");
  if (rc) return rc;
  const int tile_w = f.tile_w, tile_h = f.tile_h;
  MGS_REQUIRE(checkpoint_interval == 0 || (checkpoint_interval >= 64 && (checkpoint_interval & (checkpoint_interval - 1)) == 0),
              "rasterize_bwd_det: checkpoint_interval %d is not a power of two >= 64", checkpoint_interval);
  const size_t raster_ws = mgs::rasterize_bwd_det_workspace_bytes(channels, v_means2d_abs != nullptr, isect_capacity, tile_w,
                                                                  tile_h, checkpoint_interval);
  const BwdWs ws(n, channels, raster_ws);
  if (!workspace) {
    *workspace_bytes = ws.total;
    return MGS_OK;
  }
  if (*workspace_bytes < ws.total)
    return mgs::set_error(MGS_ERR_WORKSPACE_TOO_SMALL, "render_frames_backward: workspace %zu < %zu bytes", *workspace_bytes, ws.total);
  MGS_REQUIRE(viewmats && Ks && render && alphas && v_render && state && v_means && v_quats && v_scales && v_sh_coeffs &&
                  v_opacities, "render_frames_backward: null pointer");
  MGS_REQUIRE(((reinterpret_cast<uintptr_t>(workspace) | reinterpret_cast<uintptr_t>(state)) & 255u) == 0,
              "render_frames_backward: workspace and state must be 256-byte aligned");
  const bool own_opac = antialiased != 0 || f.raw;
  const TrainState st(n, width, height, channels, isect_capacity, own_opac, checkpoint_interval);
  char* w = static_cast<char*>(workspace);
  const size_t n_px = (size_t)width * height;
  hipStream_t hs = (hipStream_t)stream;
  for (int c = 0; c < n_cams; ++c) {
    const char* s = static_cast<const char*>(state) + st.total * (size_t)c;
    auto F = [&](int f) { return reinterpret_cast<const float*>(s + st.at[f]); };
    auto I = [&](int f) { return reinterpret_cast<const int32_t*>(s + st.at[f]); };
    const float* opac = own_opac ? F(TF_OPAC) : opacities;
    float* g_m2d = v_means2d ? v_means2d + 2 * (size_t)n * c : reinterpret_cast<float*>(w + ws.v_means2d);
    float* g_abs = v_means2d_abs ? v_means2d_abs + 2 * (size_t)n * c : nullptr;
    float* g_con = reinterpret_cast<float*>(w + ws.v_conics);
    float* g_feat = reinterpret_cast<float*>(w + ws.v_feats);
    float* g_opac = (!own_opac && c == 0) ? v_opacities : reinterpret_cast<float*>(w + ws.v_opac);
    const float* frame = render + n_px * channels * c;
    const bool ed = (flags & MGS_RASTER_EXPECTED_LAST) != 0;
    size_t rw = raster_ws;
    rc = mgs_rasterize_bwd_det(n, F(TF_MEANS2D), F(TF_CONICS), F(TF_FEATS), opac, F(TF_SPLATS),
                               backgrounds ? backgrounds + (size_t)channels * c : nullptr, channels, width, height, tile_w,
                               tile_h, I(TF_OFFSETS), I(TF_FLATTEN), alphas + n_px * c, I(TF_LAST_IDS),
                               v_render + n_px * channels * c, v_alphas ? v_alphas + n_px * c : nullptr, ed ? frame : nullptr,
                               I(TF_PAIR_INFO), I(TF_ORDER), isect_capacity, checkpoint_interval ? frame : nullptr,
                               checkpoint_interval ? F(TF_CKPT) : nullptr, checkpoint_interval, MGS_RASTER_BWD_SPLAT_SLOTS, g_m2d, g_abs, g_con, g_feat,
                               g_opac, w + ws.raster, &rw, stream);
    if (rc) return rc;
    rc = mgs_project_color_bwd(n, means, quats, scales, opacities, sh_degree, coeff_stride, sh_coeffs,
                               viewmats + 16 * (size_t)c, Ks + 9 * (size_t)c, width, height, eps2d, I(TF_RADII), F(TF_CONICS),
                               antialiased, channels, F(TF_FEATS), g_feat, g_m2d, g_con, nullptr,
                               own_opac ? g_opac : nullptr, v_means, v_quats, v_scales, v_sh_coeffs,
                               own_opac ? v_opacities : nullptr, v_viewmats ? v_viewmats + 16 * (size_t)c : nullptr,
                               c > 0 ? 1 : 0, f.camera_model | (f.raw ? MGS_PARAMS_RAW : 0), stream);
    if (rc) return rc;
    if (!own_opac && n > 0 && c > 0)
      hipLaunchKernelGGL(add_rows_kernel, dim3(mgs::div_up((unsigned)n, 256u)), dim3(256), 0, hs, (size_t)n, g_opac, v_opacities, 0);
  }
  return mgs::check_launch("render_frames_backward");
}
```

### robosimgs_amd/csrc/projection.hip

```cpp
#include "mgs_common.h"
#include "mgs_math.h"
#include "sh_staging.h"
#include "tile_rect.h"

namespace mgs {
namespace {

constexpr int kBlock = 64;
constexpr int kWave = kShWave;

__device__ __forceinline__ void load3(const float* p, float v[3]) {
  v[0] = p[0]; v[1] = p[1]; v[2] = p[2];
}

template <int CAM>
__global__ __launch_bounds__(kBlock) void projection_fwd_kernel(
    int n, const float* __restrict__ means, const float* __restrict__ quats,
    const float* __restrict__ scales, const float* __restrict__ viewmat,
    const float* __restrict__ Kmat, float W, float H, float eps2d, float near_plane,
    float far_plane, float radius_clip, int32_t* __restrict__ radii,
    float* __restrict__ means2d, float* __restrict__ depths, float* __restrict__ conics,
    float* __restrict__ compensations, const float* __restrict__ opacities, int radius_rule,
    int32_t* __restrict__ radii_y) {
  int g = blockIdx.x * kBlock + threadIdx.x;
  if (g >= n) return;
  CameraParams cam = load_camera(viewmat, Kmat);
  float m[3], s[3], q[4];
  load3(means + 3 * (size_t)g, m);
  load3(scales + 3 * (size_t)g, s);
  float4 qq = reinterpret_cast<const float4*>(quats)[g];
  q[0] = qq.x; q[1] = qq.y; q[2] = qq.z; q[3] = qq.w;
  Projected p = project_gaussian<CAM>(m, q, s, cam, W, H, eps2d, near_plane, far_plane, radius_clip, radius_rule,
                                      opacities != nullptr, opacities ? opacities[g] : 1.f, compensations != nullptr);
  radii[g] = p.radius;
  if (radii_y) radii_y[g] = p.radius_y;
  reinterpret_cast<float2*>(means2d)[g] = make_float2(p.mean2d[0], p.mean2d[1]);
  depths[g] = p.depth;
  conics[3 * (size_t)g + 0] = p.conic[0];
  conics[3 * (size_t)g + 1] = p.conic[1];
  conics[3 * (size_t)g + 2] = p.conic[2];
  if (compensations) compensations[g] = p.compensation;
}

template <int DEG>
__device__ __forceinline__ void sh_dot(const float dir[3], const float* c , float rgb[3]) {
  constexpr int KC = (DEG + 1) * (DEG + 1);
  float n2 = dir[0] * dir[0] + dir[1] * dir[1] + dir[2] * dir[2];
  float inv = n2 > 0.f ? 1.0f / sqrtf(n2) : 0.f;
  float Y[KC];
  sh_basis(DEG, dir[0] * inv, dir[1] * inv, dir[2] * inv, Y);
  float r = 0.f, g = 0.f, b = 0.f;
#pragma unroll
  for (int k = 0; k < KC; ++k) {
    r += Y[k] * c[3 * k + 0];
    g += Y[k] * c[3 * k + 1];
    b += Y[k] * c[3 * k + 2];
  }
  rgb[0] = r; rgb[1] = g; rgb[2] = b;
}

template <int DEG, bool STAGED>
__device__ __forceinline__ void fetch_sh_row(const float* __restrict__ coeffs, int stride_f,
                                             int g, int g0, int n, bool active,
                                             unsigned long long wave_mask, float4* lds,
                                             float* c) {
  constexpr int KC = (DEG + 1) * (DEG + 1);
  if constexpr (STAGED) {
    const unsigned lane = threadIdx.x & (kWave - 1);
    sh_rows_to_lds(coeffs, g0, n, wave_mask, lds);
    __syncthreads();
    constexpr int NF4 = (KC * 3 + 3) / 4;
#pragma unroll
    for (int j = 0; j < NF4; ++j) {
      float4 v = lds[lane * kShPitchF4 + j];
      c[4 * j + 0] = v.x;
      if (4 * j + 1 < KC * 3) c[4 * j + 1] = v.y;
      if (4 * j + 2 < KC * 3) c[4 * j + 2] = v.z;
      if (4 * j + 3 < KC * 3) c[4 * j + 3] = v.w;
    }
  } else {
    if (active) {
      const float* row = coeffs + (size_t)g * stride_f;
#pragma unroll
      for (int k = 0; k < KC * 3; ++k) c[k] = row[k];
    } else {
#pragma unroll
      for (int k = 0; k < KC * 3; ++k) c[k] = 0.f;
    }
  }
}

constexpr int sh_reg_floats(int deg) { return (((deg + 1) * (deg + 1) * 3 + 3) / 4) * 4; }

template <int DEG, bool STAGED>
__global__ __launch_bounds__(kBlock) void sh_fwd_kernel(
    int n, int stride_f, const float* __restrict__ dirs, const float* __restrict__ coeffs,
    const uint8_t* __restrict__ masks, float* __restrict__ colors) {
  __shared__ float4 lds[STAGED ? (kBlock / kWave) * kWave * kShPitchF4 : 1];
  int g = blockIdx.x * kBlock + threadIdx.x;
  bool active = g < n && (masks == nullptr || masks[g] != 0);
  unsigned long long wave_mask = ballot(active);
  int g0 = blockIdx.x * kBlock + (threadIdx.x & ~(kWave - 1));
  float c[sh_reg_floats(DEG)];
  fetch_sh_row<DEG, STAGED>(coeffs, stride_f, g, g0, n, active, wave_mask,
                            lds + (threadIdx.x / kWave) * kWave * kShPitchF4, c);
  if (g >= n) return;
  float rgb[3] = {0.f, 0.f, 0.f};
  if (active) {
    float d[3];
    load3(dirs + 3 * (size_t)g, d);
    sh_dot<DEG>(d, c, rgb);
  }
  colors[3 * (size_t)g + 0] = rgb[0];
  colors[3 * (size_t)g + 1] = rgb[1];
  colors[3 * (size_t)g + 2] = rgb[2];
}

template <int DEG, bool STAGED, int RULE, int CAM>
__global__ __launch_bounds__(kBlock) void project_color_fwd_kernel(
    int n, const float* __restrict__ means, const float* __restrict__ quats,
    const float* __restrict__ scales, const float* __restrict__ opacities, int stride_f,
    const float* __restrict__ coeffs, const float* __restrict__ viewmat,
    const float* __restrict__ Kmat, float W, float H, float eps2d, float near_plane,
    float far_plane, float radius_clip, int32_t* __restrict__ radii,
    float* __restrict__ means2d, float* __restrict__ depths, float* __restrict__ conics,
    float* __restrict__ opac_out, int feat_stride, float* __restrict__ feats,
    float4* __restrict__ splats, uint2* __restrict__ bin_info, uint32_t* __restrict__ bin_sums,
    int bin_tight, int tile_w, int tile_h, int32_t* __restrict__ radii_y, int params) {
  __shared__ float4 lds[STAGED ? (kBlock / kWave) * kWave * kShPitchF4 : 1];
  int g = blockIdx.x * kBlock + threadIdx.x;
  CameraParams cam = load_camera(viewmat, Kmat);
  float m[3] = {0.f, 0.f, 0.f};
  float o = 1.f;
  const bool aa = opac_out != nullptr && !(params & MGS_PARAMS_OPAC_PLAIN);
  Projected p;
  p.radius = 0;
  if (g < n) {
    float s[3], q[4];
    load3(means + 3 * (size_t)g, m);
    load3(scales + 3 * (size_t)g, s);
    if (opacities) o = opacities[g];
    if (params & MGS_PARAMS_RAW) {
      s[0] = activate_scale(s[0]); s[1] = activate_scale(s[1]); s[2] = activate_scale(s[2]);
      o = activate_opacity(o);
    }
    float4 qq = reinterpret_cast<const float4*>(quats)[g];
    q[0] = qq.x; q[1] = qq.y; q[2] = qq.z; q[3] = qq.w;
    if (RULE == MGS_RADIUS_CLASSIC)
      p = project_gaussian<CAM>(m, q, s, cam, W, H, eps2d, near_plane, far_plane, radius_clip);
    else
      p = project_gaussian<CAM>(m, q, s, cam, W, H, eps2d, near_plane, far_plane, radius_clip, RULE, opacities != nullptr,
                                o, aa);
    if (radii) radii[g] = p.radius;
    if (RULE != MGS_RADIUS_CLASSIC && radii_y) radii_y[g] = p.radius_y;
    if (means2d) reinterpret_cast<float2*>(means2d)[g] = make_float2(p.mean2d[0], p.mean2d[1]);
    depths[g] = p.depth;
    if (conics) {
      conics[3 * (size_t)g + 0] = p.conic[0];
      conics[3 * (size_t)g + 1] = p.conic[1];
      conics[3 * (size_t)g + 2] = p.conic[2];
    }
    if (opac_out) opac_out[g] = aa ? o * p.compensation : o;
  }
  bool active = p.radius > 0;
  if (bin_info) {
    uint2 info = make_uint2(kEmptyTileRect, 0u);
    if (active) {
      TileRect r = RULE == MGS_RADIUS_CLASSIC
                       ? tile_rect(p.mean2d[0], p.mean2d[1], p.radius, (float)MGS_TILE_SIZE, tile_w, tile_h)
                       : tile_rect(p.mean2d[0], p.mean2d[1], p.radius, p.radius_y, (float)MGS_TILE_SIZE, tile_w, tile_h);
      if (bin_tight)
        r = tighten_rect(r, p.mean2d[0], p.mean2d[1], p.conic[0], p.conic[1], p.conic[2],
                         o * (aa ? p.compensation : 1.f), (float)MGS_TILE_SIZE);
      info = pack_tile_rect(r);
    }
    if (g < n) bin_info[g] = info;
    uint32_t c = info.y;
#pragma unroll
    for (int d = 32; d >= 1; d >>= 1) c += __shfl_xor(c, d);
    if ((threadIdx.x & (kWave - 1)) == 0 && g < n) bin_sums[g / kWave] = c;
  }
  unsigned long long wave_mask = ballot(active);
  int g0 = blockIdx.x * kBlock + (threadIdx.x & ~(kWave - 1));
  float c[sh_reg_floats(DEG)];
  fetch_sh_row<DEG, STAGED>(coeffs, stride_f, g, g0, n, active, wave_mask,
                            lds + (threadIdx.x / kWave) * kWave * kShPitchF4, c);
  if (g >= n) return;
  float rgb[3] = {0.f, 0.f, 0.f};
  if (active) {
    float campos[3], d[3];
    camera_position(cam, campos);
    d[0] = m[0] - campos[0]; d[1] = m[1] - campos[1]; d[2] = m[2] - campos[2];
    sh_dot<DEG>(d, c, rgb);
    rgb[0] = fmaxf(rgb[0] + 0.5f, 0.f);
    rgb[1] = fmaxf(rgb[1] + 0.5f, 0.f);
    rgb[2] = fmaxf(rgb[2] + 0.5f, 0.f);
  }
  if (splats && active) {
    float op = opacities ? o * (aa ? p.compensation : 1.f) : 0.f;
    splats[3 * (size_t)g + 0] = make_float4(p.mean2d[0], p.mean2d[1], p.conic[0], p.conic[1]);
    splats[3 * (size_t)g + 1] = make_float4(p.conic[2], op, rgb[0], rgb[1]);
    splats[3 * (size_t)g + 2] = make_float4(rgb[2], feat_stride == 4 ? p.depth : 0.f, 0.f, 0.f);
  }
  if (!feats) return;
  if (feat_stride == 4) {
    reinterpret_cast<float4*>(feats)[g] = make_float4(rgb[0], rgb[1], rgb[2], p.depth);
  } else {
    feats[3 * (size_t)g + 0] = rgb[0];
    feats[3 * (size_t)g + 1] = rgb[1];
    feats[3 * (size_t)g + 2] = rgb[2];
  }
}

}
}

using namespace mgs;

extern "C" int mgs_projection_fwd(int n, const float* means, const float* quats,
                                  const float* scales, const float* viewmat, const float* K,
                                  int width, int height, float eps2d, float near_plane,
                                  float far_plane, float radius_clip, int32_t* radii,
                                  float* means2d, float* depths, float* conics,
                                  float* compensations, const float* opacities, int radius_rule,
                                  int32_t* radii_y, int camera_model, mgs_stream_t stream) {
  MGS_REQUIRE(n >= 0 && width > 0 && height > 0, "projection_fwd: bad sizes n=%d %dx%d", n, width, height);
  MGS_REQUIRE(camera_model >= MGS_CAMERA_PINHOLE && camera_model <= MGS_CAMERA_FISHEYE,
              "projection_fwd: camera_model %d is not MGS_CAMERA_PINHOLE, _ORTHO or _FISHEYE", camera_model);
  if (n == 0) return MGS_OK;
  MGS_REQUIRE(means && quats && scales && viewmat && K && radii && means2d && depths && conics,
              "projection_fwd: null pointer");
  MGS_REQUIRE(radius_rule == MGS_RADIUS_CLASSIC || radius_rule == MGS_RADIUS_OPACITY_AWARE,
              "projection_fwd: radius_rule %d is neither MGS_RADIUS_CLASSIC nor MGS_RADIUS_OPACITY_AWARE", radius_rule);
  MGS_REQUIRE(radius_rule == MGS_RADIUS_CLASSIC || radii_y, "projection_fwd: the per-axis radius rule needs radii_y");
  with_camera(camera_model, [&](auto cam) {
    hipLaunchKernelGGL(projection_fwd_kernel<decltype(cam)::value>, dim3(div_up(n, kBlock)), dim3(kBlock), 0,
                       (hipStream_t)stream, n, means, quats, scales, viewmat, K, (float)width, (float)height, eps2d,
                       near_plane, far_plane, radius_clip, radii, means2d, depths, conics, compensations, opacities,
                       radius_rule, radii_y);
  });
  return check_launch("projection_fwd");
}

extern "C" int mgs_sh_fwd(int n, int degree, int coeff_stride, const float* dirs,
                          const float* coeffs, const uint8_t* masks, float* colors,
                          mgs_stream_t stream) {
  MGS_REQUIRE(n >= 0 && degree >= 0 && degree <= 3, "sh_fwd: degree %d not in 0..3", degree);
  MGS_REQUIRE(coeff_stride >= (degree + 1) * (degree + 1), "sh_fwd: %d coefficients < (degree+1)^2", coeff_stride);
  if (n == 0) return MGS_OK;
  MGS_REQUIRE(dirs && coeffs && colors, "sh_fwd: null pointer");
  dim3 grid(div_up(n, kBlock)), block(kBlock);
  hipStream_t s = (hipStream_t)stream;
  int sf = coeff_stride * 3;
  bool staged = coeff_stride == 16 && degree >= 2;
  with_sh_degree(degree, [&](auto d) {
    with_bool(staged, [&](auto st) {
      constexpr int D = decltype(d)::value;
      if constexpr (D >= 2 || !decltype(st)::value)
        hipLaunchKernelGGL((sh_fwd_kernel<D, decltype(st)::value>), grid, block, 0, s, n, sf, dirs, coeffs, masks, colors);
    });
  });
  return check_launch("sh_fwd");
}

extern "C" int mgs_project_color_fwd(int n, const float* means, const float* quats,
                                     const float* scales, const float* opacities,
                                     int sh_degree, int coeff_stride, const float* sh_coeffs,
                                     const float* viewmat, const float* K, int width,
                                     int height, float eps2d, float near_plane,
                                     float far_plane, float radius_clip, int32_t* radii,
                                     float* means2d, float* depths, float* conics,
                                     float* opac_out, int feat_stride, float* feats,
                                     float* splats, int bin_flags, uint32_t* bin_info,
                                     uint32_t* bin_sums, int32_t* radii_y, mgs_stream_t stream) {
  const int bin_tight = bin_flags & MGS_BIN_TIGHT;
  const bool per_axis = (bin_flags & MGS_BIN_RADIUS_OPACITY_AWARE) != 0;
  MGS_REQUIRE((bin_flags & (MGS_BIN_CAMERA_ORTHO | MGS_BIN_CAMERA_FISHEYE)) != (MGS_BIN_CAMERA_ORTHO | MGS_BIN_CAMERA_FISHEYE),
              "project_color_fwd: bin_flags sets both MGS_BIN_CAMERA_ORTHO and MGS_BIN_CAMERA_FISHEYE");
  const int cam_model = bin_camera_model(bin_flags);
  const int params = bin_flags & (MGS_PARAMS_RAW | MGS_PARAMS_OPAC_PLAIN);
  MGS_REQUIRE(!(params & MGS_PARAMS_RAW) || opacities,
              "project_color_fwd: MGS_PARAMS_RAW needs opacities (the logits), got NULL");
  MGS_REQUIRE(!(params & MGS_PARAMS_OPAC_PLAIN) || ((params & MGS_PARAMS_RAW) && opac_out),
              "project_color_fwd: MGS_PARAMS_OPAC_PLAIN comes with MGS_PARAMS_RAW and opac_out");
  MGS_REQUIRE(n >= 0 && width > 0 && height > 0, "project_color_fwd: bad sizes");
  MGS_REQUIRE(sh_degree >= 0 && sh_degree <= 3, "project_color_fwd: sh_degree %d not in 0..3", sh_degree);
  MGS_REQUIRE(coeff_stride >= (sh_degree + 1) * (sh_degree + 1), "project_color_fwd: coeff_stride too small");
  MGS_REQUIRE(feat_stride == 3 || feat_stride == 4, "project_color_fwd: feat_stride must be 3 or 4");
  if (n == 0) return MGS_OK;
  MGS_REQUIRE(means && quats && scales && sh_coeffs && viewmat && K && depths, "project_color_fwd: null pointer");
  MGS_REQUIRE((radii && means2d && conics && feats) || (splats && bin_info),
              "project_color_fwd: radii / means2d / conics / feats may be NULL only when splats and bin_info are given");
  MGS_REQUIRE(!opac_out || opacities, "project_color_fwd: opac_out needs opacities");
  MGS_REQUIRE(!splats || opacities, "project_color_fwd: splats needs opacities");
  MGS_REQUIRE((bin_info == nullptr) == (bin_sums == nullptr), "project_color_fwd: bin_info and bin_sums come together");
  MGS_REQUIRE(!(bin_info && bin_tight) || opacities, "project_color_fwd: tight tile bounds need opacities");
  MGS_REQUIRE(!per_axis || !radii || radii_y, "project_color_fwd: the per-axis radius rule writes radii_y beside radii");
  const int tile_w = (width + MGS_TILE_SIZE - 1) / MGS_TILE_SIZE, tile_h = (height + MGS_TILE_SIZE - 1) / MGS_TILE_SIZE;
  MGS_REQUIRE(!bin_info || (tile_w <= 1023 && tile_h <= 1023), "project_color_fwd: tile grid exceeds 1023x1023");
  dim3 grid(div_up(n, kBlock)), block(kBlock);
  hipStream_t s = (hipStream_t)stream;
  int sf = coeff_stride * 3;
  bool staged = coeff_stride == 16 && sh_degree >= 2;
  with_sh_degree(sh_degree, [&](auto d) {
    with_bool(staged, [&](auto st) {
      with_radius_rule(per_axis, [&](auto rule) {
        with_camera(cam_model, [&](auto cam) {
          constexpr int D = decltype(d)::value;
          if constexpr (D >= 2 || !decltype(st)::value)
            hipLaunchKernelGGL((project_color_fwd_kernel<D, decltype(st)::value, decltype(rule)::value, decltype(cam)::value>),
                               grid, block, 0, s, n, means, quats, scales, opacities, sf, sh_coeffs, viewmat, K,
                               (float)width, (float)height, eps2d, near_plane, far_plane, radius_clip, radii, means2d,
                               depths, conics, opac_out, feat_stride, feats, reinterpret_cast<float4*>(splats),
                               reinterpret_cast<uint2*>(bin_info), bin_sums, bin_tight, tile_w, tile_h, radii_y, params);
        });
      });
    });
  });
  return check_launch("project_color_fwd");
}
```

### robosimgs_amd/csrc/raster_common.h

```cpp
#ifndef MGS_RASTER_COMMON_H_
#define MGS_RASTER_COMMON_H_

#include "mgs_common.h"

namespace mgs {

constexpr float kAlphaMin = 1.0f / 255.0f;
constexpr float kAlphaMax = 0.999f;
constexpr float kTStop = 1e-4f;
constexpr int kQueue = 64;

struct QuadRect { float x0, x1, y0, y1; };

__device__ __forceinline__ float edge_min_sigma(float e, float wu, float wv, float b,
                                                float inv_wv, float lo, float hi) {
  float v = fminf(fmaxf(-b * e * inv_wv, lo), hi);
  return 0.5f * (wu * e * e + wv * v * v) + b * e * v;
}

__device__ __forceinline__ float rect_min_sigma(float mx, float my, float a, float b, float c,
                                                float inv_a, float inv_c, const QuadRect& r) {
  float lx = r.x0 - mx, hx = r.x1 - mx, ly = r.y0 - my, hy = r.y1 - my;
  if (lx <= 0.f && hx >= 0.f && ly <= 0.f && hy >= 0.f) return 0.f;
  float s0 = edge_min_sigma(lx, a, c, b, inv_c, ly, hy);
  float s1 = edge_min_sigma(hx, a, c, b, inv_c, ly, hy);
  float s2 = edge_min_sigma(ly, c, a, b, inv_a, lx, hx);
  float s3 = edge_min_sigma(hy, c, a, b, inv_a, lx, hx);
  return fminf(fminf(s0, s1), fminf(s2, s3));
}

__device__ __forceinline__ unsigned quadrant_mask(float mx, float my, float a, float b, float c,
                                                  float opac, float tile_x, float tile_y) {
  if (!(opac >= kAlphaMin)) return 0u;
  float thr = 0.6931471805599453f * __builtin_amdgcn_logf(255.0f * opac);
  float inv_a = __builtin_amdgcn_rcpf(a), inv_c = __builtin_amdgcn_rcpf(c);
  float fx = fmaxf(fabsf(tile_x - mx), fabsf(tile_x + 16.f - mx));
  float fy = fmaxf(fabsf(tile_y - my), fabsf(tile_y + 16.f - my));
  float slack = 0.05f + 4e-6f * (fabsf(a) + fabsf(c) + 2.f * fabsf(b)) * (fx * fx + fy * fy);
  float lim = thr + slack;
  unsigned m = 0;
#pragma unroll
  for (int k = 0; k < 4; ++k) {
    QuadRect r;
    r.x0 = tile_x + 8.f * (k & 1) + 0.5f;
    r.x1 = r.x0 + 7.f;
    r.y0 = tile_y + 8.f * (k >> 1) + 0.5f;
    r.y1 = r.y0 + 7.f;
    float s = rect_min_sigma(mx, my, a, b, c, inv_a, inv_c, r);
    if (!(s > lim)) m |= 1u << k;
  }
  return m;
}

__device__ __forceinline__ bool sigma_sign_is_safe(float a, float b, float c) {
  const float tr = a + c;
  return a > 0.f && c > 0.f && fmaf(a, c, -b * b) >= 1e-4f * tr * tr;
}

__device__ __forceinline__ float pair_power(float dx, float dy, float A, float B, float C, float L) {
  return fmaf(dx, fmaf(B, dy, A * dx), fmaf(C * dy, dy, L));
}
__device__ __forceinline__ float pair_power_sign(float dx, float dy, float A, float B, float C) {
  return fmaf(dx, fmaf(B, dy, A * dx), (C * dy) * dy);
}
struct PolyCoef { float q0, q1, q2; };
__device__ __forceinline__ PolyCoef poly_coefs(float m_x, float m_y, float A, float B, float C, float L) {
  PolyCoef q;
  q.q0 = pair_power(m_x, m_y, A, B, C, L);
  q.q1 = -fmaf(2.f * A, m_x, B * m_y);
  q.q2 = -fmaf(2.f * C, m_y, B * m_x);
  return q;
}
struct PixelPoly { float x, y, xx, xy, yy; };
__device__ __forceinline__ PixelPoly pixel_poly(float x, float y) { return PixelPoly{x, y, x * x, x * y, y * y}; }
__device__ __forceinline__ float pair_power_poly(const PixelPoly& p, float q0, float q1, float q2, float A, float B,
                                                 float C) {
  return fmaf(C, p.yy, fmaf(B, p.xy, fmaf(A, p.xx, fmaf(q2, p.y, fmaf(q1, p.x, q0)))));
}

constexpr float kSafeOpacity = 0.998f;
constexpr float kSafeConicTrace = 8.0f;
__device__ __forceinline__ bool entry_is_safe(float a, float b, float c, float op) {
  return sigma_sign_is_safe(a, b, c) && op <= kSafeOpacity && a + c <= kSafeConicTrace;
}

__host__ __device__ constexpr size_t ckpt_units(uint32_t capacity, int n_tiles, int shift) {
  return ((size_t)capacity >> shift) + (size_t)n_tiles + 1;
}
__host__ __device__ constexpr size_t ckpt_header_floats(int n_tiles) { return ((size_t)n_tiles * 4 + 255) / 256 * 256; }
__device__ __forceinline__ size_t ckpt_unit(int start, int tile, int seg, int shift) {
  return (size_t)(start >> shift) + (size_t)tile + (size_t)seg;
}

typedef float mgs_f4 __attribute__((ext_vector_type(4)));
__device__ __forceinline__ void lds_read_3f4(const float4* pa, const float4* pb, const float4* pc, float4& a, float4& b,
                                             float4& c) {
  mgs_f4 va = *reinterpret_cast<const mgs_f4*>(pa), vb = *reinterpret_cast<const mgs_f4*>(pb),
         vc = *reinterpret_cast<const mgs_f4*>(pc);
  asm volatile("" : "+v"(va), "+v"(vb), "+v"(vc));
  a = make_float4(va.x, va.y, va.z, va.w);
  b = make_float4(vb.x, vb.y, vb.z, vb.w);
  c = make_float4(vc.x, vc.y, vc.z, vc.w);
}

__device__ __forceinline__ float wave_reduce_to_lane63(float v) {
  int i;
#define MGS_DPP_ADD(CTRL, RMASK)                                                               \
  i = __builtin_amdgcn_update_dpp(0, __float_as_int(v), CTRL, RMASK, 0xf, false);              \
  v += __int_as_float(i);
  MGS_DPP_ADD(0xB1, 0xf)
  MGS_DPP_ADD(0x4E, 0xf)
  MGS_DPP_ADD(0x141, 0xf)
  MGS_DPP_ADD(0x140, 0xf)
  MGS_DPP_ADD(0x142, 0xa)
  MGS_DPP_ADD(0x143, 0xc)
#undef MGS_DPP_ADD
  return v;
}


__device__ __forceinline__ float dpp_f(float x, int ctrl) {
  switch (ctrl) {
    case 0xB1: return __int_as_float(__builtin_amdgcn_update_dpp(0, __float_as_int(x), 0xB1, 0xf, 0xf, false));
    case 0x4E: return __int_as_float(__builtin_amdgcn_update_dpp(0, __float_as_int(x), 0x4E, 0xf, 0xf, false));
    case 0x128: return __int_as_float(__builtin_amdgcn_update_dpp(0, __float_as_int(x), 0x128, 0xf, 0xf, false));
    default: return __int_as_float(__builtin_amdgcn_update_dpp(0, __float_as_int(x), 0x104, 0xf, 0xf, false));
  }
}
constexpr int kDppXor1 = 0xB1, kDppXor2 = 0x4E, kDppRor8 = 0x128, kDppShl4 = 0x104;

template <int V>
__device__ __forceinline__ float wave_reduce_scatter(const float* v, unsigned lane) {
  static_assert(V == 8 || V == 4 || V == 2 || V == 1, "V must be 8, 4, 2 or 1");
  const bool b0 = lane & 1u, b1 = lane & 2u, b3 = lane & 8u;
  float t;
  if constexpr (V == 8) {
    float w[4], u[2];
#pragma unroll
    for (int i = 0; i < 4; ++i) w[i] = (b0 ? v[i + 4] : v[i]) + dpp_f(b0 ? v[i] : v[i + 4], kDppXor1);
#pragma unroll
    for (int i = 0; i < 2; ++i) u[i] = (b1 ? w[i + 2] : w[i]) + dpp_f(b1 ? w[i] : w[i + 2], kDppXor2);
    t = (b3 ? u[1] : u[0]) + dpp_f(b3 ? u[0] : u[1], kDppRor8);
  } else if constexpr (V == 4) {
    float u[2];
#pragma unroll
    for (int i = 0; i < 2; ++i) u[i] = (b0 ? v[i + 2] : v[i]) + dpp_f(b0 ? v[i] : v[i + 2], kDppXor1);
    t = (b1 ? u[1] : u[0]) + dpp_f(b1 ? u[0] : u[1], kDppXor2);
    t += dpp_f(t, kDppRor8);
  } else if constexpr (V == 2) {
    t = (b0 ? v[1] : v[0]) + dpp_f(b0 ? v[0] : v[1], kDppXor1);
    t += dpp_f(t, kDppXor2);
    t += dpp_f(t, kDppRor8);
  } else {
    t = v[0] + dpp_f(v[0], kDppXor1);
    t += dpp_f(t, kDppXor2);
    t += dpp_f(t, kDppRor8);
  }
  t += dpp_f(t, kDppShl4);
  t += __shfl_down(t, 16);
  t += __shfl_down(t, 32);
  return t;
}
template <int V>
__device__ __forceinline__ int wave_reduce_scatter_index(unsigned lane) {
  if (lane & ~0xBu) return -1;
  const int b0 = lane & 1, b1 = (lane >> 1) & 1, b3 = (lane >> 3) & 1;
  if (V == 8) return b3 + 2 * b1 + 4 * b0;
  if (V == 4) return b3 ? -1 : b1 + 2 * b0;
  if (V == 2) return (b3 || b1) ? -1 : b0;
  return lane == 0 ? 0 : -1;
}

}
#endif
```

### robosimgs_amd/csrc/tile_rect.h

```cpp
#ifndef MGS_TILE_RECT_H_
#define MGS_TILE_RECT_H_

#include "mgs_common.h"

namespace mgs {

struct TileRect { int x0, y0, w, h; };

__device__ __forceinline__ TileRect tile_rect(float mx, float my, int radius_x, int radius_y, float tile_size,
                                              int tile_w, int tile_h) {
  TileRect r;
  float trx = (float)radius_x / tile_size, try_ = (float)radius_y / tile_size;
  float tx = mx / tile_size, ty = my / tile_size;
  int x0 = min(max(0, (int)floorf(tx - trx)), tile_w);
  int x1 = min(max(0, (int)ceilf(tx + trx)), tile_w);
  int y0 = min(max(0, (int)floorf(ty - try_)), tile_h);
  int y1 = min(max(0, (int)ceilf(ty + try_)), tile_h);
  r.x0 = x0; r.y0 = y0; r.w = x1 - x0; r.h = y1 - y0;
  return r;
}
__device__ __forceinline__ TileRect tile_rect(float mx, float my, int radius, float tile_size,
                                              int tile_w, int tile_h) {
  return tile_rect(mx, my, radius, radius, tile_size, tile_w, tile_h);
}

__device__ __forceinline__ TileRect tighten_rect(TileRect r, float mx, float my, float a, float b,
                                                 float c, float opac, float tile_size) {
  if (!(opac >= 1.0f / 255.0f)) { r.w = 0; r.h = 0; return r; }
  const float w = b * b, e = fmaf(-b, b, w), f = fmaf(a, c, -w);
  const float det = f + e;
  if (!(det > 0.f) || !(a > 0.f) || !(c > 0.f)) return r;
  const float inv_det = 1.0f / det;
  const float sxx = c * inv_det, syy = a * inv_det;
  const float thr = __logf(255.0f * opac);
  const float e2 = 2.0f * (thr + 0.05f) * (sxx + syy);
  const float slack = 0.05f + 8e-6f * (fabsf(a) + fabsf(c) + 2.f * fabsf(b)) * (e2 + 512.f);
  const float lim = 2.0f * (thr + slack);
  const float ex = sqrtf(lim * sxx) * 1.0001f + 0.01f;
  const float ey = sqrtf(lim * syy) * 1.0001f + 0.01f;
  const float plx = ceilf(mx - ex - 0.5f), phx = floorf(mx + ex - 0.5f);
  const float ply = ceilf(my - ey - 0.5f), phy = floorf(my + ey - 0.5f);
  if (!(phx >= plx) || !(phy >= ply)) {
    if (phx < plx || phy < ply) { r.w = 0; r.h = 0; }
    return r;
  }
  const int x0 = max(r.x0, (int)fmaxf(floorf(plx / tile_size), -1.f));
  const int y0 = max(r.y0, (int)fmaxf(floorf(ply / tile_size), -1.f));
  const int x1 = min(r.x0 + r.w, (int)fminf(floorf(phx / tile_size), 65535.f) + 1);
  const int y1 = min(r.y0 + r.h, (int)fminf(floorf(phy / tile_size), 65535.f) + 1);
  if (x1 <= x0 || y1 <= y0) { r.w = 0; r.h = 0; return r; }
  r.x0 = x0; r.y0 = y0; r.w = x1 - x0; r.h = y1 - y0;
  return r;
}

__device__ __forceinline__ uint2 pack_tile_rect(const TileRect& r) {
  return make_uint2((uint32_t)r.x0 | ((uint32_t)r.y0 << 10) | ((uint32_t)max(r.w, 1) << 20),
                    (uint32_t)(r.w * r.h));
}
constexpr uint32_t kEmptyTileRect = 1u << 20;

}
#endif
```

### robosimgs_amd/ops.py

```python
from __future__ import annotations

import ctypes
from typing import Optional, Tuple

import torch
from torch import Tensor

from . import _lib
from ._lib import check, ptr, require_device, sized_call, stream_handle

TILE_SIZE = 16


def _f32c(t: Optional[Tensor]) -> Optional[Tensor]:
    if t is None:
        return None
    if t.dtype != torch.float32:
        t = t.float()
    return t.contiguous()


RADIUS_RULES = {"classic": 0, "opacity_aware": 1}


def radius_rule_id(radius_rule) -> int:
    if radius_rule not in RADIUS_RULES:
        raise ValueError(f"radius_rule {radius_rule!r} not in {tuple(RADIUS_RULES)}")
    return RADIUS_RULES[radius_rule]


CAMERA_MODELS = {"pinhole": 0, "ortho": 1, "fisheye": 2}

RASTER_EXPECTED_LAST, RASTER_LATENCY = 1, 2
FRAMES_CLASSIC_BOUNDS, FRAMES_RADIUS_OPACITY_AWARE = 4, 8
FRAMES_CAMERA_ORTHO, FRAMES_CAMERA_FISHEYE = 16, 32
BIN_TIGHT, BIN_RADIUS_OPACITY_AWARE = 1, 2
BIN_CAMERA_ORTHO, BIN_CAMERA_FISHEYE = 4, 8
RASTER_BWD_RECORDS_ONLY, RASTER_BWD_SPLAT_SLOTS = 1, 2
PARAMS_RAW = 64
PARAMS_OPAC_PLAIN = 128
CAMERA_BIN_FLAGS = {0: 0, 1: BIN_CAMERA_ORTHO, 2: BIN_CAMERA_FISHEYE}
CAMERA_FRAME_FLAGS = {0: 0, 1: FRAMES_CAMERA_ORTHO, 2: FRAMES_CAMERA_FISHEYE}


def frames_flags(expected_last, latency, tight, per_axis, camera, raw=False) -> int:
    return ((RASTER_EXPECTED_LAST if expected_last else 0) | (RASTER_LATENCY if latency else 0)
            | (0 if tight else FRAMES_CLASSIC_BOUNDS) | (FRAMES_RADIUS_OPACITY_AWARE if per_axis else 0)
            | CAMERA_FRAME_FLAGS[int(camera)] | (PARAMS_RAW if raw else 0))


def camera_model_id(camera_model) -> int:
    if camera_model not in CAMERA_MODELS:
        raise ValueError(f"camera_model {camera_model!r} not in {tuple(CAMERA_MODELS)}")
    return CAMERA_MODELS[camera_model]


def radii_x(radii):
    return radii if radii is None or radii.dim() == 1 else radii[0]


def radii_meta(radii):
    return radii if radii is None or radii.dim() == 1 else radii.t()


def projection_fwd_raw(means, quats, scales, viewmat, K, width, height, eps2d, near_plane,
                       far_plane, radius_clip, calc_compensations, opacities=None, radius_rule=0, camera=0):
    n = means.shape[0]
    dev = means.device
    radii = torch.empty((2, n) if radius_rule else (n,), dtype=torch.int32, device=dev)
    means2d = torch.empty(n, 2, dtype=torch.float32, device=dev)
    depths = torch.empty(n, dtype=torch.float32, device=dev)
    conics = torch.empty(n, 3, dtype=torch.float32, device=dev)
    comp = torch.empty(n, dtype=torch.float32, device=dev) if calc_compensations else None
    check(_lib.lib().mgs_projection_fwd(n, ptr(means), ptr(quats), ptr(scales), ptr(viewmat),
                                        ptr(K), width, height, eps2d, near_plane, far_plane,
                                        radius_clip, ptr(radii_x(radii)), ptr(means2d), ptr(depths),
                                        ptr(conics), ptr(comp), ptr(opacities) if radius_rule else None,
                                        int(radius_rule), ptr(radii[1]) if radius_rule else None, int(camera),
                                        stream_handle()),
          "mgs_projection_fwd")
    return radii, means2d, depths, conics, comp


def project_color_fwd_raw(means, quats, scales, opacities, sh_degree, sh_coeffs, viewmat, K,
                          width, height, eps2d, near_plane, far_plane, radius_clip,
                          antialiased, with_depth, want_splats=False, bin_seed=None, lean=False, per_axis=False, camera=0,
                          raw=False):
    n = means.shape[0]
    dev = means.device
    if lean and not (want_splats and bin_seed is not None):
        raise ValueError("lean=True needs want_splats=True and a bin_seed")
    stride = 4 if with_depth else 3
    radii = means2d = conics = feats = None
    if not lean:
        radii = torch.empty((2, n) if per_axis else (n,), dtype=torch.int32, device=dev)
        means2d = torch.empty(n, 2, dtype=torch.float32, device=dev)
        conics = torch.empty(n, 3, dtype=torch.float32, device=dev)
        feats = torch.empty(n, stride, dtype=torch.float32, device=dev)
    depths = torch.empty(n, dtype=torch.float32, device=dev)
    keep_plain = bool(raw) and not antialiased and not lean
    opac = torch.empty(n, dtype=torch.float32, device=dev) if (antialiased or keep_plain) else None
    splats = torch.empty(n, 12, dtype=torch.float32, device=dev) if want_splats else None
    seed = None
    if bin_seed is not None and n > 0:
        seed = (torch.empty(n, 2, dtype=torch.int32, device=dev),
                torch.empty(max(1, -(-n // 64)), dtype=torch.int32, device=dev))
    check(_lib.lib().mgs_project_color_fwd(
        n, ptr(means), ptr(quats), ptr(scales), ptr(opacities), sh_degree, sh_coeffs.shape[1],
        ptr(sh_coeffs), ptr(viewmat), ptr(K), width, height, eps2d, near_plane, far_plane,
        radius_clip, ptr(radii_x(radii)), ptr(means2d), ptr(depths), ptr(conics), ptr(opac), stride,
        ptr(feats), ptr(splats),
        (BIN_TIGHT if bin_seed == "tight" else 0) | (BIN_RADIUS_OPACITY_AWARE if per_axis else 0) | CAMERA_BIN_FLAGS[int(camera)]
        | (PARAMS_RAW if raw else 0) | (PARAMS_OPAC_PLAIN if keep_plain else 0),
        ptr(seed[0]) if seed else None,
        ptr(seed[1]) if seed else None, ptr(radii[1]) if (per_axis and radii is not None) else None, stream_handle()),
        "mgs_project_color_fwd")
    out = (radii, means2d, depths, conics, opac, feats)
    if want_splats or bin_seed is not None:
        out = out + (splats,)
    if bin_seed is not None:
        out = out + (seed,)
    return out


def project_color_bwd_raw(means, quats, scales, opacities, sh_degree, sh_coeffs, viewmat, K, width, height, eps2d,
                          radii, conics, antialiased, feats, v_feats, v_means2d, v_conics, v_opac_aa, v_means, v_quats,
                          v_scales, v_sh, v_opacities, v_viewmat=None, accumulate=False, camera=0, raw=False):
    check(_lib.lib().mgs_project_color_bwd(
        means.shape[0], ptr(means), ptr(quats), ptr(scales), ptr(opacities), sh_degree, sh_coeffs.shape[1], ptr(sh_coeffs),
        ptr(viewmat), ptr(K), width, height, eps2d, ptr(radii_x(radii)), ptr(conics), int(antialiased), feats.shape[1],
        ptr(feats), ptr(v_feats), ptr(v_means2d), ptr(v_conics), None, ptr(v_opac_aa), ptr(v_means), ptr(v_quats),
        ptr(v_scales), ptr(v_sh), ptr(v_opacities), ptr(v_viewmat), int(accumulate),
        int(camera) | (PARAMS_RAW if raw else 0), stream_handle()), "mgs_project_color_bwd")


class TileLists:
    __slots__ = ("n_isect", "tile_ids", "flatten_ids", "tile_offsets", "tiles_per_gauss",
                 "isect_ids", "status", "capacity", "pair_info", "group_order", "splat_slots")


def _tag_splat_slots(tl: TileLists, splats) -> None:
    tl.splat_slots = object()
    splats._mgs_splat_slots = tl.splat_slots


def isect_tiles_raw(means2d, radii, depths, tile_w, tile_h, capacity: int, cam_id=0, n_cams=1,
                    want_isect_ids=False, want_tiles_per_gauss=True,
                    want_pair_info=False, conics=None, opacities=None, seed=None,
                    want_tile_ids=True, want_group_order=True, splats=None) -> TileLists:
    n = depths.shape[0]
    dev = depths.device
    out = TileLists()
    out.capacity = int(capacity)
    out.n_isect = torch.empty(1, dtype=torch.int32, device=dev)
    out.status = torch.empty(1, dtype=torch.int32, device=dev)
    out.tile_ids = torch.empty(capacity, dtype=torch.int32, device=dev) if want_tile_ids else None
    out.flatten_ids = torch.empty(capacity, dtype=torch.int32, device=dev)
    out.tile_offsets = torch.empty(tile_w * tile_h + 1, dtype=torch.int32, device=dev)
    out.tiles_per_gauss = (torch.empty(n, dtype=torch.int32, device=dev)
                           if want_tiles_per_gauss else None)
    out.isect_ids = torch.empty(capacity, dtype=torch.int64, device=dev) if want_isect_ids else None
    out.pair_info = torch.empty(n, 4, dtype=torch.int32, device=dev) if want_pair_info else None
    out.group_order = (torch.empty((tile_w * tile_h + 3) // 4, dtype=torch.int32, device=dev) if want_group_order else None)
    annotate = splats is not None and want_pair_info
    args = [n, ptr(means2d), ptr(radii_x(radii)), ptr(radii[1]) if (radii is not None and radii.dim() == 2) else None,
            ptr(depths), ptr(conics), ptr(opacities), TILE_SIZE,
            tile_w, tile_h, cam_id, n_cams,
            capacity, ptr(out.tiles_per_gauss), ptr(out.n_isect), ptr(out.tile_ids),
            ptr(out.flatten_ids), ptr(out.isect_ids), ptr(out.tile_offsets), ptr(out.pair_info),
            ptr(out.group_order), ptr(out.status), ptr(seed[0]) if seed else None, ptr(seed[1]) if seed else None,
            ptr(splats) if annotate else None]
    out.splat_slots = False
    if annotate:
        _tag_splat_slots(out, splats)
    sized_call(_lib.lib().mgs_isect_tiles, args, dev, cached=True)
    return out


def _frames_call(means, quats, scales, opacities, sh_degree, sh_coeffs, viewmats, Ks, width, height, eps2d, near_plane,
                 far_plane, radius_clip, antialiased, with_depth, capacity, backgrounds, flags, out):
    dev = means.device
    C, ch = viewmats.shape[0], 4 if with_depth else 3
    if out is None:
        out = (torch.empty(C, height, width, ch, dtype=torch.float32, device=dev),
               torch.empty(C, height, width, dtype=torch.float32, device=dev))
    args = [means.shape[0], ptr(means), ptr(quats), ptr(scales), ptr(opacities), int(sh_degree), sh_coeffs.shape[1],
            ptr(sh_coeffs), C, ptr(viewmats), ptr(Ks), int(width), int(height), eps2d, near_plane, far_plane, radius_clip,
            int(bool(antialiased)), ch, flags, ptr(backgrounds), int(capacity)]
    return out[0], out[1], args


def render_frames_raw(means, quats, scales, opacities, sh_degree, sh_coeffs, viewmats, Ks, width, height,
                      eps2d, near_plane, far_plane, radius_clip, antialiased, with_depth, capacity,
                      backgrounds=None, expected_last=False, latency=False, out=None, tight=True, per_axis=False,
                      dataset=None, float_frame=True, camera=0, raw=False):
    dev = means.device
    C = viewmats.shape[0]
    render, alphas, args = _frames_call(means, quats, scales, opacities, sh_degree, sh_coeffs, viewmats, Ks, width, height,
                                        eps2d, near_plane, far_plane, radius_clip, antialiased, with_depth, capacity,
                                        backgrounds, frames_flags(expected_last, latency, tight, per_axis, camera, raw), out)
    n_isect = torch.empty(C, dtype=torch.int32, device=dev)
    status = torch.empty(C, dtype=torch.int32, device=dev)
    args += [ptr(render) if (float_frame or dataset is None) else None,
             ptr(alphas) if (float_frame or dataset is None) else None, ptr(n_isect), ptr(status)]
    ds = dataset_args(dataset, C, height, width, dev)
    args += list(ds[:4])
    sized_call(_lib.lib().mgs_render_frames, args, dev, cached=True)
    return render, alphas, n_isect, status


def checkpoint_buffer(capacity: int, tile_w: int, tile_h: int, channels: int, interval: int, device) -> Tensor:
    n = _lib.lib().mgs_raster_checkpoint_floats(int(capacity), tile_w, tile_h, channels, int(interval))
    if n == 0:
        raise ValueError(f"checkpoint interval {interval} is not a power of two >= 64")
    return torch.empty(n, dtype=torch.float32, device=device)


TRAIN_FIELDS = ("radii", "means2d", "depths", "conics", "opac_aa", "feats", "splats", "tiles_per_gauss", "pair_info",
                "tile_ids", "flatten_ids", "tile_offsets", "group_order", "last_ids", "checkpoints", "counts", "radii_y")


class TrainState:

    def __init__(self, n, n_cams, width, height, channels, capacity, antialiased, interval, flags, device, raw=False):
        offs = (ctypes.c_size_t * len(TRAIN_FIELDS))()
        per = ctypes.c_size_t(0)
        self.raw = bool(raw)
        self.keep_opac = bool(antialiased) or self.raw
        check(_lib.lib().mgs_train_state_layout(n, width, height, channels, int(capacity), int(self.keep_opac), int(interval),
                                                offs, ctypes.byref(per)), "mgs_train_state_layout")
        self.offsets, self.per_camera = list(offs), per.value
        self.n, self.n_cams, self.width, self.height, self.channels = n, n_cams, width, height, channels
        self.capacity, self.antialiased, self.interval, self.flags = int(capacity), bool(antialiased), int(interval), flags
        self.buf = torch.empty(self.per_camera * n_cams + 256, dtype=torch.uint8, device=device)
        self.pad = (-self.buf.data_ptr()) % 256
        self.n_tiles = (-(-width // TILE_SIZE)) * (-(-height // TILE_SIZE))

    def ptr(self) -> int:
        return self.buf.data_ptr() + self.pad

    def views(self, c: int) -> dict:
        n, cap, nt = self.n, self.capacity, self.n_tiles
        shapes = {"radii": (torch.int32, (n,)), "means2d": (torch.float32, (n, 2)), "depths": (torch.float32, (n,)),
                  "conics": (torch.float32, (n, 3)), "opac_aa": (torch.float32, (n,) if self.keep_opac else (0,)),
                  "feats": (torch.float32, (n, self.channels)), "splats": (torch.float32, (n, 12)),
                  "tiles_per_gauss": (torch.int32, (n,)), "pair_info": (torch.int32, (n, 4)), "tile_ids": (torch.int32, (cap,)),
                  "flatten_ids": (torch.int32, (cap,)), "tile_offsets": (torch.int32, (nt + 1,)),
                  "group_order": (torch.int32, ((nt + 3) // 4,)), "last_ids": (torch.int32, (self.height, self.width)),
                  "counts": (torch.int32, (2,)), "radii_y": (torch.int32, (n,))}
        out = {}
        base = self.pad + self.per_camera * c
        for name, off in zip(TRAIN_FIELDS, self.offsets):
            if name not in shapes:
                continue
            dt, shape = shapes[name]
            numel = 1
            for d_ in shape:
                numel *= d_
            nbytes = numel * (4)
            out[name] = self.buf[base + off:base + off + nbytes].view(dt).view(shape)
        return out

    def tile_lists(self, c: int, v: dict = None) -> "TileLists":
        v = v or self.views(c)
        tl = TileLists()
        tl.capacity = self.capacity
        tl.n_isect, tl.status = v["counts"][0:1], v["counts"][1:2]
        tl.tile_ids, tl.flatten_ids, tl.tile_offsets = v["tile_ids"], v["flatten_ids"], v["tile_offsets"]
        tl.tiles_per_gauss, tl.pair_info, tl.group_order, tl.isect_ids = v["tiles_per_gauss"], v["pair_info"], v["group_order"], None
        tl.splat_slots = True
        return tl


def render_frames_train_raw(means, quats, scales, opacities, sh_degree, sh_coeffs, viewmats, Ks, width, height, eps2d,
                            near_plane, far_plane, radius_clip, antialiased, with_depth, capacity, interval,
                            backgrounds=None, expected_last=False, latency=True, tight=True, out=None, per_axis=False,
                            camera=0, raw=False):
    flags = frames_flags(expected_last, latency, tight, per_axis, camera, raw)
    render, alphas, args = _frames_call(means, quats, scales, opacities, sh_degree, sh_coeffs, viewmats, Ks, width, height,
                                        eps2d, near_plane, far_plane, radius_clip, antialiased, with_depth, capacity,
                                        backgrounds, flags, out)
    st = TrainState(means.shape[0], viewmats.shape[0], width, height, 4 if with_depth else 3, capacity, antialiased, interval,
                    flags, means.device, raw=raw)
    args += [int(interval), ptr(render), ptr(alphas), st.ptr()]
    sized_call(_lib.lib().mgs_render_frames_train, args, means.device, cached=True)
    return render, alphas, st


def render_frames_backward_raw(means, quats, scales, opacities, sh_degree, sh_coeffs, viewmats, Ks, eps2d, backgrounds, st,
                               render, alphas, v_render, v_alphas, absgrad=False, want_viewmats=False, raw=False):
    if bool(raw) != bool(st.flags & PARAMS_RAW):
        raise ValueError(f"raw={bool(raw)} but the TrainState was rendered with raw={bool(st.flags & PARAMS_RAW)}")
    dev = means.device
    C, n = viewmats.shape[0], means.shape[0]
    v_means, v_quats, v_scales = torch.empty_like(means), torch.empty_like(quats), torch.empty_like(scales)
    v_sh, v_opac = torch.empty_like(sh_coeffs), torch.empty_like(opacities)
    v_vm = torch.zeros_like(viewmats) if want_viewmats else None
    v_m2d = torch.empty(C, n, 2, dtype=torch.float32, device=dev)
    v_abs = torch.empty(C, n, 2, dtype=torch.float32, device=dev) if absgrad else None
    args = [n, ptr(means), ptr(quats), ptr(scales), ptr(opacities), int(sh_degree), sh_coeffs.shape[1], ptr(sh_coeffs), C,
            ptr(viewmats), ptr(Ks), st.width, st.height, eps2d, int(st.antialiased), st.channels, st.flags, ptr(backgrounds),
            st.capacity, st.interval, ptr(render), ptr(alphas), ptr(v_render), ptr(v_alphas), st.ptr(), ptr(v_means),
            ptr(v_quats), ptr(v_scales), ptr(v_sh), ptr(v_opac), ptr(v_vm), ptr(v_m2d), ptr(v_abs)]
    sized_call(_lib.lib().mgs_render_frames_backward, args, dev, cached=False)
    return v_means, v_quats, v_scales, v_sh, v_opac, v_vm, v_m2d, v_abs


def dataset_args(dataset, n_frames=None, height=None, width=None, device=None):
    if dataset is None:
        return None, None, 0, None, None
    import numpy as np
    rgba, dist, K = dataset
    if rgba.dtype != torch.uint8 or not rgba.is_contiguous():
        raise ValueError("dataset rgba must be a contiguous uint8 tensor [..., H, W, 4]")
    if dist is not None and (not dist.is_contiguous() or dist.dtype not in (torch.float16, torch.float32, torch.float64)):
        raise ValueError("dataset distance must be a contiguous float16 / float32 / float64 tensor [..., H, W, 1]")
    require_device(rgba, dist)
    if device is not None and any(x is not None and x.device != device for x in (rgba, dist)):
        raise ValueError(f"dataset buffers must live on {device}, the device the frame is rendered on")
    if n_frames is not None:
        n_px = int(n_frames) * int(height) * int(width)
        if rgba.numel() != n_px * 4:
            raise ValueError(f"dataset rgba holds {rgba.numel()} bytes, {n_frames} frame(s) of {width}x{height} need {n_px * 4} "
                             f"([{n_frames},{height},{width},4] uint8)")
        if dist is not None and dist.numel() != n_px:
            raise ValueError(f"dataset distance holds {dist.numel()} values, {n_frames} frame(s) of {width}x{height} need {n_px} "
                             f"([{n_frames},{height},{width},1])")
    if dist is not None and K is None:
        raise ValueError("a dataset distance plane needs K (the 3x3 intrinsics the cameras of the call share)")
    kinv = np.ascontiguousarray(np.linalg.inv(np.asarray(K, dtype=np.float64).reshape(3, 3))) if dist is not None else None
    dtype_id = {torch.float64: 1, torch.float16: 2}.get(dist.dtype, 0) if dist is not None else 0
    return ptr(rgba), ptr(dist), dtype_id, (kinv.ctypes.data if kinv is not None else None), kinv


def rasterize_fwd_raw(means2d, conics, feats, opacities, background, width, height, tile_w,
                      tile_h, tile_offsets, flatten_ids, out=None, track_last=True, splats=None,
                      expected_last=False, latency=False, group_order=None, channels=None,
                      checkpoints=None, checkpoint_interval=0, dataset=None):
    src = means2d if means2d is not None else splats
    n = src.shape[0]
    ch = int(channels) if channels is not None else feats.shape[-1]
    dev = src.device
    if out is None:
        render = torch.empty(height, width, ch, dtype=torch.float32, device=dev)
        alphas = torch.empty(height, width, dtype=torch.float32, device=dev)
        last_ids = (torch.empty(height, width, dtype=torch.int32, device=dev) if track_last
                    else None)
    else:
        render, alphas, last_ids = out
    ds = dataset_args(dataset, 1, height, width, dev)
    check(_lib.lib().mgs_rasterize_fwd(n, ptr(means2d), ptr(conics), ptr(feats), ptr(opacities),
                                       ptr(splats), ptr(background), ch, width, height, tile_w, tile_h,
                                       ptr(tile_offsets), ptr(flatten_ids), ptr(group_order),
                                       (RASTER_EXPECTED_LAST if expected_last else 0) | (RASTER_LATENCY if latency else 0),
                                       ptr(render), ptr(alphas), ptr(last_ids), ptr(checkpoints),
                                       int(checkpoint_interval), *ds[:4], stream_handle()),
          "mgs_rasterize_fwd")
    return render, alphas, last_ids


def rasterize_bwd_raw(means2d, conics, feats, opacities, background, width, height, tile_w,
                      tile_h, tile_offsets, flatten_ids, alphas, last_ids, v_render, v_alphas,
                      absgrad=False, accum=None):
    n = means2d.shape[0]
    ch = feats.shape[-1]
    dev = means2d.device
    if accum is None:
        v_means2d = torch.zeros(n, 2, dtype=torch.float32, device=dev)
        v_conics = torch.zeros(n, 3, dtype=torch.float32, device=dev)
        v_feats = torch.zeros(n, ch, dtype=torch.float32, device=dev)
        v_opac = torch.zeros(n, dtype=torch.float32, device=dev)
        v_abs = torch.zeros(n, 2, dtype=torch.float32, device=dev) if absgrad else None
    else:
        v_means2d, v_conics, v_feats, v_opac, v_abs = accum
    check(_lib.lib().mgs_rasterize_bwd(
        n, ptr(means2d), ptr(conics), ptr(feats), ptr(opacities), ptr(background), ch, width,
        height, tile_w, tile_h, ptr(tile_offsets), ptr(flatten_ids), ptr(alphas), ptr(last_ids),
        ptr(v_render), ptr(v_alphas), ptr(v_means2d), ptr(v_abs), ptr(v_conics), ptr(v_feats),
        ptr(v_opac), stream_handle()), "mgs_rasterize_bwd")
    return v_means2d, v_conics, v_feats, v_opac, v_abs


def _splat_slots_valid(tl, splats) -> bool:
    tag = getattr(tl, "splat_slots", False)
    if splats is None or not tag:
        return False
    return tag is True or getattr(splats, "_mgs_splat_slots", None) is tag


def rasterize_bwd_det_raw(means2d, conics, feats, opacities, background, width, height, tile_w,
                          tile_h, tl: "TileLists", alphas, last_ids, v_render, v_alphas,
                          absgrad=False, splats=None, canary_bytes=0, expected_render=None,
                          render_out=None, checkpoints=None, checkpoint_interval=0, records_only=False):
    n = means2d.shape[0]
    ch = feats.shape[-1]
    dev = means2d.device
    v_means2d = torch.empty(n, 2, dtype=torch.float32, device=dev)
    v_conics = torch.empty(n, 3, dtype=torch.float32, device=dev)
    v_feats = torch.empty(n, ch, dtype=torch.float32, device=dev)
    v_opac = torch.empty(n, dtype=torch.float32, device=dev)
    v_abs = torch.empty(n, 2, dtype=torch.float32, device=dev) if absgrad else None
    args = [n, ptr(means2d), ptr(conics), ptr(feats), ptr(opacities), ptr(splats), ptr(background),
            ch, width, height, tile_w, tile_h, ptr(tl.tile_offsets), ptr(tl.flatten_ids), ptr(alphas),
            ptr(last_ids), ptr(v_render), ptr(v_alphas), ptr(expected_render), ptr(tl.pair_info),
            ptr(getattr(tl, "group_order", None)), tl.capacity,
            ptr(render_out), ptr(checkpoints), int(checkpoint_interval),
            (RASTER_BWD_RECORDS_ONLY if records_only else 0) | (RASTER_BWD_SPLAT_SLOTS if _splat_slots_valid(tl, splats) else 0),
            ptr(v_means2d), ptr(v_abs), ptr(v_conics), ptr(v_feats), ptr(v_opac)]
    canary = sized_call(_lib.lib().mgs_rasterize_bwd_det, args, dev, cached=False, canary_bytes=canary_bytes)
    if canary_bytes:
        return v_means2d, v_conics, v_feats, v_opac, v_abs, canary
    return v_means2d, v_conics, v_feats, v_opac, v_abs


class _Projection(torch.autograd.Function):
    @staticmethod
    def forward(ctx, means, quats, scales, viewmats, Ks, width, height, eps2d, near_plane,
                far_plane, radius_clip, calc_compensations, opacities=None, radius_rule=0, camera=0):
        C = viewmats.shape[0]
        outs = [projection_fwd_raw(means, quats, scales, viewmats[c], Ks[c], width, height,
                                   eps2d, near_plane, far_plane, radius_clip,
                                   calc_compensations, opacities, radius_rule, camera) for c in range(C)]
        radii_out = torch.stack([radii_meta(o[0]) for o in outs])
        radii = torch.stack([radii_x(o[0]) for o in outs])
        means2d = torch.stack([o[1] for o in outs])
        depths = torch.stack([o[2] for o in outs])
        conics = torch.stack([o[3] for o in outs])
        comps = torch.stack([o[4] for o in outs]) if calc_compensations else None
        ctx.save_for_backward(means, quats, scales, viewmats, Ks, radii, conics, comps)
        ctx.dims = (width, height, eps2d, camera)
        ctx.mark_non_differentiable(radii_out)
        return radii_out, means2d, depths, conics, comps

    @staticmethod
    def backward(ctx, _v_radii, v_means2d, v_depths, v_conics, v_comps):
        means, quats, scales, viewmats, Ks, radii, conics, comps = ctx.saved_tensors
        width, height, eps2d, camera = ctx.dims
        n, C = means.shape[0], viewmats.shape[0]
        v_means = torch.zeros_like(means)
        v_quats = torch.zeros_like(quats)
        v_scales = torch.zeros_like(scales)
        want_view = ctx.needs_input_grad[3]
        v_viewmats = torch.zeros_like(viewmats) if want_view else None
        v_means2d, v_depths, v_conics = _f32c(v_means2d), _f32c(v_depths), _f32c(v_conics)
        v_comps = _f32c(v_comps) if comps is not None else None
        for c in range(C):
            check(_lib.lib().mgs_projection_bwd(
                n, ptr(means), ptr(quats), ptr(scales), ptr(viewmats[c]), ptr(Ks[c]), width,
                height, eps2d, ptr(radii[c]), ptr(conics[c]),
                ptr(comps[c]) if comps is not None else None,
                ptr(v_means2d[c]), ptr(v_depths[c]), ptr(v_conics[c]),
                ptr(v_comps[c]) if v_comps is not None else None, ptr(v_means), ptr(v_quats),
                ptr(v_scales), ptr(v_viewmats[c]) if want_view else None, int(camera), stream_handle()),
                "mgs_projection_bwd")
        return (v_means, v_quats, v_scales, v_viewmats, None, None, None, None, None, None,
                None, None, None, None, None)


def fully_fused_projection(means: Tensor, covars: Optional[Tensor], quats: Tensor,
                           scales: Tensor, viewmats: Tensor, Ks: Tensor, width: int,
                           height: int, eps2d: float = 0.3, near_plane: float = 0.01,
                           far_plane: float = 1e10, radius_clip: float = 0.0,
                           packed: bool = False, sparse_grad: bool = False,
                           calc_compensations: bool = False, opacities: Optional[Tensor] = None,
                           radius_rule: str = "classic", camera_model: str = "pinhole"
                           ) -> Tuple[Tensor, Tensor, Tensor, Tensor, Optional[Tensor]]:
    if covars is not None:
        raise NotImplementedError("precomputed covariances are not supported; pass quats+scales")
    if packed:
        raise NotImplementedError("packed=True is not supported (nerfstudio uses packed=False)")
    require_device(means, quats, scales, viewmats, Ks)
    means, quats, scales = _f32c(means), _f32c(quats), _f32c(scales)
    viewmats, Ks = _f32c(viewmats), _f32c(Ks)
    if means.dim() != 2 or means.shape[1] != 3 or quats.shape != (means.shape[0], 4) \
            or scales.shape != means.shape:
        raise ValueError("expected means [N,3], quats [N,4], scales [N,3]")
    if viewmats.dim() != 3 or viewmats.shape[1:] != (4, 4) or Ks.shape != (viewmats.shape[0], 3, 3):
        raise ValueError("expected viewmats [C,4,4], Ks [C,3,3]")
    rule = radius_rule_id(radius_rule)
    camera = camera_model_id(camera_model)
    if opacities is not None:
        require_device(opacities)
        opacities = _f32c(opacities.detach())
        if opacities.shape != (means.shape[0],):
            raise ValueError("expected opacities [N]")
    return _Projection.apply(means, quats, scales, viewmats, Ks, int(width), int(height),
                             float(eps2d), float(near_plane), float(far_plane),
                             float(radius_clip), bool(calc_compensations), opacities if rule else None, rule, camera)


class _SphericalHarmonics(torch.autograd.Function):
    @staticmethod
    def forward(ctx, degree, dirs, coeffs, masks):
        n = dirs.shape[0]
        colors = torch.empty(n, 3, dtype=torch.float32, device=dirs.device)
        check(_lib.lib().mgs_sh_fwd(n, degree, coeffs.shape[1], ptr(dirs), ptr(coeffs), ptr(masks),
                                    ptr(colors), stream_handle()), "mgs_sh_fwd")
        ctx.save_for_backward(dirs, coeffs, masks)
        ctx.degree = degree
        return colors

    @staticmethod
    def backward(ctx, v_colors):
        dirs, coeffs, masks = ctx.saved_tensors
        n = dirs.shape[0]
        v_coeffs = torch.empty_like(coeffs)
        v_dirs = torch.empty_like(dirs) if ctx.needs_input_grad[1] else None
        check(_lib.lib().mgs_sh_bwd(n, ctx.degree, coeffs.shape[1], ptr(dirs), ptr(coeffs),
                                    ptr(masks), ptr(_f32c(v_colors)), ptr(v_coeffs), ptr(v_dirs),
                                    stream_handle()), "mgs_sh_bwd")
        return None, v_dirs, v_coeffs, None


def spherical_harmonics(degrees_to_use: int, dirs: Tensor, coeffs: Tensor,
                        masks: Optional[Tensor] = None) -> Tensor:
    require_device(dirs, coeffs, masks)
    if not 0 <= degrees_to_use <= 3:
        raise ValueError(f"degrees_to_use={degrees_to_use} outside 0..3")
    if coeffs.shape[-2] < (degrees_to_use + 1) ** 2:
        raise ValueError("coeffs holds fewer than (degrees_to_use+1)^2 coefficients")
    if dirs.shape[:-1] != coeffs.shape[:-2] or dirs.shape[-1] != 3 or coeffs.shape[-1] != 3:
        raise ValueError("expected dirs [...,3] and coeffs [...,K,3] with equal batch dims")
    batch = dirs.shape[:-1]
    d = _f32c(dirs).reshape(-1, 3)
    c = _f32c(coeffs).reshape(-1, coeffs.shape[-2], 3)
    m = None
    if masks is not None:
        m = masks.reshape(-1).to(torch.uint8).contiguous()
    return _SphericalHarmonics.apply(int(degrees_to_use), d, c, m).reshape(*batch, 3)


@torch.no_grad()
def isect_tiles(means2d: Tensor, radii: Tensor, depths: Tensor, tile_size: int,
                tile_width: int, tile_height: int, sort: bool = True, packed: bool = False,
                n_cameras: Optional[int] = None, camera_ids: Optional[Tensor] = None,
                gaussian_ids: Optional[Tensor] = None) -> Tuple[Tensor, Tensor, Tensor]:
    if packed or not sort:
        raise NotImplementedError("only packed=False, sort=True is supported")
    if tile_size != TILE_SIZE:
        raise NotImplementedError(f"tile_size must be {TILE_SIZE}")
    require_device(means2d, radii, depths)
    C, N = means2d.shape[0], means2d.shape[1]
    means2d, depths = _f32c(means2d), _f32c(depths)
    radii = radii.to(torch.int32)
    if radii.dim() == 3:
        if radii.shape[-1] != 2:
            raise ValueError("expected radii [C,N] or [C,N,2]")
        radii = radii.transpose(1, 2)
    radii = radii.contiguous()
    tpg, keys, ids = [], [], []
    for c in range(C):
        cap = max(1, int(_upper_bound_isects(radii[c], tile_width, tile_height)))
        tl = isect_tiles_raw(means2d[c], radii[c], depths[c], tile_width, tile_height, cap, c, C,
                             want_isect_ids=True)
        n = int(tl.n_isect.item())
        tpg.append(tl.tiles_per_gauss)
        keys.append(tl.isect_ids[:n])
        ids.append(tl.flatten_ids[:n] + c * N if c else tl.flatten_ids[:n])
    return torch.stack(tpg), torch.cat(keys), torch.cat(ids)


def _upper_bound_isects(radii_c: Tensor, tile_w: int, tile_h: int) -> int:
    rx = radii_x(radii_c).clamp_min(0).to(torch.float32)
    ry = rx if radii_c.dim() == 1 else radii_c[1].clamp_min(0).to(torch.float32)
    side_x = torch.floor(2.0 * rx / TILE_SIZE) + 2.0
    side_y = torch.floor(2.0 * ry / TILE_SIZE) + 2.0
    per = torch.minimum(side_x.clamp_max(tile_w) * side_y.clamp_max(tile_h),
                        torch.tensor(float(tile_w * tile_h), device=rx.device))
    return int(torch.where(radii_x(radii_c) > 0, per, torch.zeros_like(per)).sum().item())


@torch.no_grad()
def isect_offset_encode(isect_ids: Tensor, n_cameras: int, tile_width: int,
                        tile_height: int) -> Tensor:
    require_device(isect_ids)
    isect_ids = isect_ids.contiguous()
    out = torch.empty(n_cameras, tile_height, tile_width, dtype=torch.int32,
                      device=isect_ids.device)
    check(_lib.lib().mgs_isect_offset_encode(isect_ids.numel(), ptr(isect_ids), n_cameras,
                                             tile_width, tile_height, ptr(out), stream_handle()),
          "mgs_isect_offset_encode")
    return out


class _RasterizeToPixels(torch.autograd.Function):
    @staticmethod
    def forward(ctx, means2d, conics, colors, opacities, backgrounds, width, height,
                offsets_ext, flatten_ids, absgrad):
        C, N, ch = colors.shape
        tile_w, tile_h = -(-width // TILE_SIZE), -(-height // TILE_SIZE)
        n_tiles = tile_w * tile_h
        dev = means2d.device
        render = torch.empty(C, height, width, ch, dtype=torch.float32, device=dev)
        alphas = torch.empty(C, height, width, dtype=torch.float32, device=dev)
        last_ids = torch.empty(C, height, width, dtype=torch.int32, device=dev)
        for c in range(C):
            rasterize_fwd_raw(means2d.view(C * N, 2), conics.view(C * N, 3),
                              colors.view(C * N, ch), opacities.view(C * N),
                              backgrounds[c] if backgrounds is not None else None, width, height,
                              tile_w, tile_h, offsets_ext[c * n_tiles:], flatten_ids,
                              out=(render[c], alphas[c], last_ids[c]))
        ctx.save_for_backward(means2d, conics, colors, opacities, backgrounds, offsets_ext,
                              flatten_ids, alphas, last_ids)
        ctx.dims = (width, height, tile_w, tile_h, absgrad)
        return render, alphas.unsqueeze(-1)

    @staticmethod
    def backward(ctx, v_render, v_alphas):
        (means2d, conics, colors, opacities, backgrounds, offsets_ext, flatten_ids, alphas,
         last_ids) = ctx.saved_tensors
        width, height, tile_w, tile_h, absgrad = ctx.dims
        C, N, ch = colors.shape
        n_tiles = tile_w * tile_h
        dev = means2d.device
        v_render = _f32c(v_render)
        v_alphas = _f32c(v_alphas).reshape(C, height, width)
        acc = (torch.zeros(C * N, 2, device=dev), torch.zeros(C * N, 3, device=dev),
               torch.zeros(C * N, ch, device=dev), torch.zeros(C * N, device=dev),
               torch.zeros(C * N, 2, device=dev) if absgrad else None)
        for c in range(C):
            rasterize_bwd_raw(means2d.view(C * N, 2), conics.view(C * N, 3),
                              colors.view(C * N, ch), opacities.view(C * N),
                              backgrounds[c] if backgrounds is not None else None, width, height,
                              tile_w, tile_h, offsets_ext[c * n_tiles:], flatten_ids, alphas[c],
                              last_ids[c], v_render[c], v_alphas[c], absgrad, accum=acc)
        v_bg = None
        if backgrounds is not None and ctx.needs_input_grad[4]:
            v_bg = (v_render * (1.0 - alphas).unsqueeze(-1)).sum(dim=(1, 2))
        if absgrad:
            means2d.absgrad = acc[4].view(C, N, 2)
        return (acc[0].view(C, N, 2), acc[1].view(C, N, 3), acc[2].view(C, N, ch),
                acc[3].view(C, N), v_bg, None, None, None, None, None)


def rasterize_to_pixels(means2d: Tensor, conics: Tensor, colors: Tensor, opacities: Tensor,
                        image_width: int, image_height: int, tile_size: int,
                        isect_offsets: Tensor, flatten_ids: Tensor,
                        backgrounds: Optional[Tensor] = None, masks: Optional[Tensor] = None,
                        packed: bool = False, absgrad: bool = False) -> Tuple[Tensor, Tensor]:
    if packed:
        raise NotImplementedError("packed=True is not supported")
    if masks is not None:
        raise NotImplementedError("tile masks are not supported")
    if tile_size != TILE_SIZE:
        raise NotImplementedError(f"tile_size must be {TILE_SIZE}")
    require_device(means2d, conics, colors, opacities, isect_offsets, flatten_ids, backgrounds)
    C, N = means2d.shape[0], means2d.shape[1]
    ch = colors.shape[-1]
    if not 1 <= ch <= 32:
        raise ValueError(f"{ch} colour channels: supported range is 1..32")
    tile_w, tile_h = -(-image_width // TILE_SIZE), -(-image_height // TILE_SIZE)
    if tuple(isect_offsets.shape) != (C, tile_h, tile_w):
        raise ValueError(f"isect_offsets shape {tuple(isect_offsets.shape)} != {(C, tile_h, tile_w)}")
    flatten_ids = flatten_ids.to(torch.int32).contiguous()
    end = torch.full((1,), flatten_ids.numel(), dtype=torch.int32, device=means2d.device)
    offsets_ext = torch.cat([isect_offsets.reshape(-1).to(torch.int32), end])
    return _RasterizeToPixels.apply(_f32c(means2d), _f32c(conics), _f32c(colors),
                                    _f32c(opacities), _f32c(backgrounds), int(image_width),
                                    int(image_height), offsets_ext, flatten_ids, bool(absgrad))
```

Measured before the change: 4375.

## Skip unreachable corner tiles of tightened rects during binning

During projection, the four corner tiles of each small tightened tile rectangle are tested against the Gaussian's opacity-scaled ellipse. Corners that cannot reach alpha threshold are flagged in the upper bits of the packed count word. The direct histogram and scatter kernels then skip emitting those tile/gaussian pairs, which shrinks intersection lists and reduces rasterizer work. The change adds per-gaussian cull math in projection and extra bookkeeping so the reported intersection count still includes the skipped pairs. The frame path enables it whenever tight binning is on.

```diff
diff --git a/include/mgs.h b/include/mgs.h
--- a/include/mgs.h
+++ b/include/mgs.h
@@ -38,6 +38,7 @@
 #define MGS_BIN_RADIUS_OPACITY_AWARE 2
 #define MGS_BIN_CAMERA_ORTHO 4
 #define MGS_BIN_CAMERA_FISHEYE 8
+#define MGS_BIN_CORNERS 0x10
 
 #define MGS_PARAMS_RAW 64
 #define MGS_PARAMS_OPAC_PLAIN 128
diff --git a/robosimgs_amd/csrc/binning.hip b/robosimgs_amd/csrc/binning.hip
--- a/robosimgs_amd/csrc/binning.hip
+++ b/robosimgs_amd/csrc/binning.hip
@@ -114,7 +114,7 @@
   const unsigned lane = threadIdx.x & 63, wave = threadIdx.x >> 6;
   int g = blockIdx.x * kBlock + threadIdx.x;
   uint2 info = g < n ? ginfo[g] : make_uint2(1u << 20, 0u);
-  uint32_t cnt = info.y;
+  uint32_t cnt = tile_rect_count(info.y);
   uint32_t incl = cnt;
 #pragma unroll
   for (int d = 1; d < 64; d <<= 1) {
@@ -150,7 +150,7 @@
   if (r < n) {
     uint2 info = ginfo[r];
     pack = info.x;
-    cnt = info.y;
+    cnt = tile_rect_count(info.y);
     if (tiles_per_gauss) tiles_per_gauss[r] = (int32_t)cnt;
   }
   uint32_t incl = cnt;
@@ -215,14 +215,20 @@
 constexpr uint32_t kCoopRect = 24;
 constexpr uint32_t kRunRect = 128;
 
-template <class F>
-__device__ __forceinline__ void for_each_tile(uint32_t pack, uint32_t cnt, uint32_t g, int tile_w, F f) {
+static_assert(kCoopRect <= 32, "tile_rect_skip_mask covers the rectangles a lane walks alone");
+__device__ __forceinline__ uint32_t lane_skip_mask(uint32_t pack, uint32_t word1) {
+  const uint32_t cnt = tile_rect_count(word1);
+  return cnt > kCoopRect ? 0u : tile_rect_skip_mask(pack >> 20, cnt, tile_rect_corners(word1));
+}
+template <bool CORNERS, class F>
+__device__ __forceinline__ void for_each_tile(uint32_t pack, uint32_t word1, uint32_t g, int tile_w, F f) {
+  const uint32_t cnt = tile_rect_count(word1);
   const bool big = cnt > kCoopRect;
   if (!big) {
-    const uint32_t w = pack >> 20;
+    const uint32_t w = pack >> 20, skip = CORNERS ? tile_rect_skip_mask(w, cnt, tile_rect_corners(word1)) : 0u;
     uint32_t t = ((pack >> 10) & 1023u) * (uint32_t)tile_w + (pack & 1023u), dx = 0;
     for (uint32_t k = 0; k < cnt; ++k) {
-      f(t + dx, g);
+      if (!((skip >> k) & 1u)) f(t + dx, g);
       if (++dx == w) { dx = 0; t += (uint32_t)tile_w; }
     }
   }
@@ -240,14 +246,15 @@
   }
 }
 
-template <class F>
-__device__ __forceinline__ void for_each_tile_run(uint32_t pack, uint32_t cnt, uint32_t g, int tile_w, int shift, F f) {
+template <bool CORNERS, class F>
+__device__ __forceinline__ void for_each_tile_run(uint32_t pack, uint32_t word1, uint32_t g, int tile_w, int shift, F f) {
+  const uint32_t cnt = tile_rect_count(word1);
   const bool big = cnt > kCoopRect;
   if (!big) {
-    const uint32_t w = pack >> 20;
+    const uint32_t w = pack >> 20, keep = CORNERS ? ~tile_rect_skip_mask(w, cnt, tile_rect_corners(word1)) : ~0u;
     uint32_t t = ((pack >> 10) & 1023u) * (uint32_t)tile_w + (pack & 1023u), dx = 0;
     for (uint32_t k = 0; k < cnt; ++k) {
-      f(t + dx, 1u, g);
+      f(t + dx, CORNERS ? (keep >> k) & 1u : 1u, g);
       if (++dx == w) { dx = 0; t += (uint32_t)tile_w; }
     }
   }
@@ -293,11 +300,14 @@
   }
 };
 
+template <bool CORNERS>
 __global__ __launch_bounds__(kDirectThreads) void direct_hist_kernel(
     int n, int chunk, const uint2* __restrict__ ginfo, int tile_w, int n_tiles, int shift,
     uint32_t* __restrict__ table, int32_t* __restrict__ tiles_per_gauss, uint32_t* __restrict__ scan_sums, uint32_t n_sums,
-    int deal_nb) {
+    int deal_nb, uint32_t* __restrict__ left_out_rows) {
   extern __shared__ uint32_t hist[];
+  __shared__ uint32_t left_out_wg;
+  if (CORNERS && threadIdx.x == 0) left_out_wg = 0u;
   if (scan_sums && blockIdx.x == gridDim.x - 1) {
     scan_blocksums_body<kDirectThreads>(n_sums, scan_sums, 0u, nullptr, nullptr);
     return;
@@ -305,6 +315,7 @@
   n_tiles = (n_tiles + (1 << shift) - 1) >> shift;
   for (int i = threadIdx.x; i < n_tiles; i += kDirectThreads) hist[i] = 0u;
   __syncthreads();
+  uint32_t left_out = 0;
   const int g0 = blockIdx.x * chunk, g1 = min(n, g0 + chunk);
   const DealtIndex gi{g0, g1, n, deal_nb};
   const int g_end = deal_nb > 0 ? g0 + chunk : g1;
@@ -318,16 +329,19 @@
 #pragma unroll
     for (int i = 0; i < kDirectPerThread; ++i) {
       const int g = gi(base, i);
-      if (g >= 0 && tiles_per_gauss) tiles_per_gauss[g] = (int32_t)info[i].y;
+      if (g >= 0 && tiles_per_gauss) tiles_per_gauss[g] = (int32_t)tile_rect_count(info[i].y);
+      if (CORNERS) left_out += (uint32_t)__popc(lane_skip_mask(info[i].x, info[i].y));
       if (shift > 0)
-        for_each_tile_run(info[i].x, info[i].y, (uint32_t)g, tile_w, shift, [&](uint32_t tile, uint32_t n_run, uint32_t) { atomicAdd(&hist[tile >> shift], n_run); });
+        for_each_tile_run<CORNERS>(info[i].x, info[i].y, (uint32_t)g, tile_w, shift, [&](uint32_t tile, uint32_t n_run, uint32_t) { atomicAdd(&hist[tile >> shift], n_run); });
       else
-        for_each_tile(info[i].x, info[i].y, (uint32_t)g, tile_w, [&](uint32_t tile, uint32_t) { atomicAdd(&hist[tile >> shift], 1u); });
-    }
-  }
+        for_each_tile<CORNERS>(info[i].x, info[i].y, (uint32_t)g, tile_w, [&](uint32_t tile, uint32_t) { atomicAdd(&hist[tile >> shift], 1u); });
+    }
+  }
+  if (CORNERS && left_out) atomicAdd(&left_out_wg, left_out);
   __syncthreads();
   uint32_t* row = table + (size_t)blockIdx.x * n_tiles;
   for (int i = threadIdx.x; i < n_tiles; i += kDirectThreads) row[i] = hist[i];
+  if (CORNERS && left_out_rows && threadIdx.x == 0) left_out_rows[blockIdx.x] = left_out_wg;
 }
 
 constexpr int kColThreads = 256, kColBins = 16, kColGroups = kColThreads / kColBins, kColKeepTraining = 32;
@@ -402,7 +416,7 @@
     uint32_t* __restrict__ flatten_ids, int32_t* __restrict__ tile_offsets,
     uint32_t* __restrict__ n_isect, uint32_t* __restrict__ status, int32_t* __restrict__ group_order,
     const uint32_t* __restrict__ scanned_sums, int4* __restrict__ pair_info, uint32_t* __restrict__ zero_word,
-    float* __restrict__ splat_slots, int deal_nb) {
+    float* __restrict__ splat_slots, int deal_nb, const uint32_t* __restrict__ left_out_rows, int n_rows) {
   extern __shared__ uint32_t cursor[];
   n_tiles = (n_tiles + (1 << shift) - 1) >> shift;
   if (group_order && blockIdx.x == gridDim.x - 1) {
@@ -424,6 +438,14 @@
     if (lane >= (unsigned)d) incl += ((unsigned long long)hi << 32) | lo;
   }
   if (lane == 63) wsum[wave] = incl;
+  __shared__ uint32_t left_out_total;
+  if (!PAIRS && blockIdx.x == 0 && left_out_rows) {
+    if (threadIdx.x == 0) left_out_total = 0u;
+    __syncthreads();
+    uint32_t v = 0;
+    for (int r = threadIdx.x; r < n_rows; r += kDirectThreads) v += left_out_rows[r];
+    if (v) atomicAdd(&left_out_total, v);
+  }
   __syncthreads();
   unsigned long long off = 0, total = 0;
 #pragma unroll
@@ -444,8 +466,9 @@
   }
   if (blockIdx.x == 0 && threadIdx.x == 0) {
     tile_offsets[n_tiles] = (int32_t)(total < capacity ? (uint32_t)total : capacity);
-    *n_isect = total > 0xffffffffull ? 0xffffffffu : (uint32_t)total;
-    *status = total > capacity ? MGS_STATUS_ISECT_OVERFLOW : 0u;
+    const unsigned long long pairs = total + ((!PAIRS && left_out_rows) ? left_out_total : 0u);
+    *n_isect = pairs > 0xffffffffull ? 0xffffffffu : (uint32_t)pairs;
+    *status = pairs > capacity ? MGS_STATUS_ISECT_OVERFLOW : 0u;
     if (zero_word) reinterpret_cast<uint4*>(zero_word)[0] = reinterpret_cast<uint4*>(zero_word)[1] = make_uint4(0u, 0u, 0u, 0u);
   }
   __syncthreads();
@@ -469,7 +492,7 @@
 #pragma unroll
       for (int i = 0; i < kDirectPerThread; ++i) {
         const int g = gi(base, i);
-        const uint32_t cnt = info[i].y;
+        const uint32_t cnt = tile_rect_count(info[i].y);
         uint32_t incl = cnt;
 #pragma unroll
         for (int d = 1; d < 64; d <<= 1) {
@@ -489,13 +512,13 @@
     for (int i = 0; i < kDirectPerThread; ++i) {
       const int g = gi(base, i);
       if (shift > 0)
-        for_each_tile_run(info[i].x, info[i].y, (uint32_t)g, tile_w, shift, [&](uint32_t tile, uint32_t n_run, uint32_t gs) {
+        for_each_tile_run<!PAIRS>(info[i].x, info[i].y, (uint32_t)g, tile_w, shift, [&](uint32_t tile, uint32_t n_run, uint32_t gs) {
           const uint32_t p = atomicAdd(&cursor[tile >> shift], n_run);
           for (uint32_t k = 0; k < n_run; ++k)
             if (p + k < capacity) flatten_ids[p + k] = gs | (((tile + k) & local_mask) << (32 - shift));
         });
       else
-      for_each_tile(info[i].x, info[i].y, (uint32_t)g, tile_w, [&](uint32_t tile, uint32_t gs) {
+      for_each_tile<!PAIRS>(info[i].x, info[i].y, (uint32_t)g, tile_w, [&](uint32_t tile, uint32_t gs) {
         const uint32_t p = atomicAdd(&cursor[tile >> shift], 1u);
         if (p < capacity) flatten_ids[p] = shift ? gs | ((tile & local_mask) << (32 - shift)) : gs;
       });
@@ -688,8 +711,13 @@
       const int bins = (n_tiles + (1 << gshift) - 1) >> gshift;
       const size_t lds = (size_t)bins * sizeof(uint32_t);
       const int deal_nb = (int)nb;
-      hipLaunchKernelGGL(direct_hist_kernel, dim3(nb + (pair_info ? 1 : 0)), dim3(kDirectThreads), lds, s, n, chunk, ginfo, tile_w,
-                         n_tiles, gshift, u32(ws.table), tiles_per_gauss, pair_info ? sums : nullptr, nsum, deal_nb);
+      static_assert(kDirectThreads * kDirectPerThread >= kSum, "left_out_rows fits the blocksums field");
+      uint32_t* left_out_rows = (seed_info && !pair_info) ? u32(ws.blocksums) : nullptr;
+      with_bool(left_out_rows != nullptr, [&](auto corners) {
+        hipLaunchKernelGGL(direct_hist_kernel<decltype(corners)::value>, dim3(nb + (pair_info ? 1 : 0)), dim3(kDirectThreads), lds, s, n,
+                           chunk, ginfo, tile_w, n_tiles, gshift, u32(ws.table), tiles_per_gauss, pair_info ? sums : nullptr, nsum,
+                           deal_nb, left_out_rows);
+      });
       if (pair_info)
         hipLaunchKernelGGL(direct_colscan_kernel<kColKeepTraining>, dim3(div_up((unsigned)bins, (unsigned)kColBins)), dim3(kColThreads), 0, s,
                            (int)nb, bins, u32(ws.table), u32(ws.tile_count));
@@ -704,7 +732,8 @@
                            u32(ws.tile_count), cap, gshift ? u32(ws.id_alt) : reinterpret_cast<uint32_t*>(flatten_ids),
                            gshift ? reinterpret_cast<int32_t*>(w + ws.group_offsets) : tile_offsets, n_isect, status,
                            order_in_scatter ? tile_group_order : nullptr, sums, reinterpret_cast<int4*>(pair_info),
-                           tile_depth_sort_long_list(w + ws.tsort, cap), pair_info ? splat_slots : nullptr, deal_nb);
+                           tile_depth_sort_long_list(w + ws.tsort, cap), pair_info ? splat_slots : nullptr, deal_nb,
+                           left_out_rows, (int)nb);
       });
     } else {
       hipLaunchKernelGGL(scan_blocksums_kernel, dim3(1), dim3(kScanThreads), 0, s, nsum, sums, cap,
diff --git a/robosimgs_amd/csrc/build.py b/robosimgs_amd/csrc/build.py
--- a/robosimgs_amd/csrc/build.py
+++ b/robosimgs_amd/csrc/build.py
@@ -11,7 +11,7 @@
 SOURCES = ["api.hip", "projection.hip", "sort.hip", "binning.hip", "tile_sort.hip", "raster_fwd.hip",
            "raster_bwd.hip", "backward.hip", "composite.hip", "points.hip", "loss.hip", "transform.hip", "frame.hip",
            "optim.hip", "refine.hip"]
-HEADERS = ["mgs_common.h", "mgs_math.h", "raster_common.h", "sh_staging.h", "tile_rect.h", "tile_order.h",
+HEADERS = ["mgs_common.h", "mgs_math.h", "raster_common.h", "sh_staging.h", "tile_cull.h", "tile_rect.h", "tile_order.h",
            "../../include/mgs.h", "../../include/mgs_optim.h",
            "../../include/mgs_refine.h"]
 LIB = os.path.join(HERE, "libmgs.so")
diff --git a/robosimgs_amd/csrc/frame.hip b/robosimgs_amd/csrc/frame.hip
--- a/robosimgs_amd/csrc/frame.hip
+++ b/robosimgs_amd/csrc/frame.hip
@@ -97,10 +97,11 @@
   int32_t* offsets = reinterpret_cast<int32_t*>(w + ws.offsets);
   int32_t* order = reinterpret_cast<int32_t*>(w + ws.order);
   const size_t n_px = (size_t)width * height;
+  const int bin_flags = f.bin_flags | ((f.bin_flags & MGS_BIN_TIGHT) ? MGS_BIN_CORNERS : 0);
   for (int c = 0; c < n_cams; ++c) {
     rc = mgs_project_color_fwd(n, means, quats, scales, opacities, sh_degree, coeff_stride, sh_coeffs,
                                viewmats + 16 * (size_t)c, Ks + 9 * (size_t)c, width, height, eps2d, near_plane, far_plane,
-                               radius_clip, nullptr, nullptr, depths, nullptr, opac_aa, channels, nullptr, splats, f.bin_flags,
+                               radius_clip, nullptr, nullptr, depths, nullptr, opac_aa, channels, nullptr, splats, bin_flags,
                                bin_info, bin_sums, nullptr, stream);
     if (rc) return rc;
     size_t iw = ws.isect_bytes;
diff --git a/robosimgs_amd/csrc/projection.hip b/robosimgs_amd/csrc/projection.hip
--- a/robosimgs_amd/csrc/projection.hip
+++ b/robosimgs_amd/csrc/projection.hip
@@ -169,13 +169,16 @@
       TileRect r = RULE == MGS_RADIUS_CLASSIC
                        ? tile_rect(p.mean2d[0], p.mean2d[1], p.radius, (float)MGS_TILE_SIZE, tile_w, tile_h)
                        : tile_rect(p.mean2d[0], p.mean2d[1], p.radius, p.radius_y, (float)MGS_TILE_SIZE, tile_w, tile_h);
-      if (bin_tight)
-        r = tighten_rect(r, p.mean2d[0], p.mean2d[1], p.conic[0], p.conic[1], p.conic[2],
-                         o * (aa ? p.compensation : 1.f), (float)MGS_TILE_SIZE);
-      info = pack_tile_rect(r);
+      const float op = o * (aa ? p.compensation : 1.f);
+      uint32_t corners = 0u;
+      if (bin_tight & MGS_BIN_TIGHT)
+        r = tighten_rect(r, p.mean2d[0], p.mean2d[1], p.conic[0], p.conic[1], p.conic[2], op, (float)MGS_TILE_SIZE);
+      if (bin_tight & MGS_BIN_CORNERS)
+        corners = unreachable_corners(r, p.mean2d[0], p.mean2d[1], p.conic[0], p.conic[1], p.conic[2], op, (float)MGS_TILE_SIZE);
+      info = pack_tile_rect(r, corners);
     }
     if (g < n) bin_info[g] = info;
-    uint32_t c = info.y;
+    uint32_t c = tile_rect_count(info.y);
 #pragma unroll
     for (int d = 32; d >= 1; d >>= 1) c += __shfl_xor(c, d);
     if ((threadIdx.x & (kWave - 1)) == 0 && g < n) bin_sums[g / kWave] = c;
@@ -273,7 +276,9 @@
                                      float* opac_out, int feat_stride, float* feats,
                                      float* splats, int bin_flags, uint32_t* bin_info,
                                      uint32_t* bin_sums, int32_t* radii_y, mgs_stream_t stream) {
-  const int bin_tight = bin_flags & MGS_BIN_TIGHT;
+  const int bin_tight = bin_flags & (MGS_BIN_TIGHT | MGS_BIN_CORNERS);
+  MGS_REQUIRE(!(bin_flags & MGS_BIN_CORNERS) || (bin_flags & MGS_BIN_TIGHT),
+              "project_color_fwd: MGS_BIN_CORNERS marks corners of the tightened rectangles: it needs MGS_BIN_TIGHT");
   const bool per_axis = (bin_flags & MGS_BIN_RADIUS_OPACITY_AWARE) != 0;
   MGS_REQUIRE((bin_flags & (MGS_BIN_CAMERA_ORTHO | MGS_BIN_CAMERA_FISHEYE)) != (MGS_BIN_CAMERA_ORTHO | MGS_BIN_CAMERA_FISHEYE),
               "project_color_fwd: bin_flags sets both MGS_BIN_CAMERA_ORTHO and MGS_BIN_CAMERA_FISHEYE");
@@ -294,7 +299,7 @@
   MGS_REQUIRE(!opac_out || opacities, "project_color_fwd: opac_out needs opacities");
   MGS_REQUIRE(!splats || opacities, "project_color_fwd: splats needs opacities");
   MGS_REQUIRE((bin_info == nullptr) == (bin_sums == nullptr), "project_color_fwd: bin_info and bin_sums come together");
-  MGS_REQUIRE(!(bin_info && bin_tight) || opacities, "project_color_fwd: tight tile bounds need opacities");
+  MGS_REQUIRE(!(bin_info && (bin_tight & MGS_BIN_TIGHT)) || opacities, "project_color_fwd: tight tile bounds need opacities");
   MGS_REQUIRE(!per_axis || !radii || radii_y, "project_color_fwd: the per-axis radius rule writes radii_y beside radii");
   const int tile_w = (width + MGS_TILE_SIZE - 1) / MGS_TILE_SIZE, tile_h = (height + MGS_TILE_SIZE - 1) / MGS_TILE_SIZE;
   MGS_REQUIRE(!bin_info || (tile_w <= 1023 && tile_h <= 1023), "project_color_fwd: tile grid exceeds 1023x1023");
diff --git a/robosimgs_amd/csrc/raster_common.h b/robosimgs_amd/csrc/raster_common.h
--- a/robosimgs_amd/csrc/raster_common.h
+++ b/robosimgs_amd/csrc/raster_common.h
@@ -2,55 +2,14 @@
 #define MGS_RASTER_COMMON_H_
 
 #include "mgs_common.h"
+#include "tile_cull.h"
 
 namespace mgs {
 
-constexpr float kAlphaMin = 1.0f / 255.0f;
 constexpr float kAlphaMax = 0.999f;
 constexpr float kTStop = 1e-4f;
 constexpr int kQueue = 64;
 
-struct QuadRect { float x0, x1, y0, y1; };
-
-__device__ __forceinline__ float edge_min_sigma(float e, float wu, float wv, float b,
-                                                float inv_wv, float lo, float hi) {
-  float v = fminf(fmaxf(-b * e * inv_wv, lo), hi);
-  return 0.5f * (wu * e * e + wv * v * v) + b * e * v;
-}
-
-__device__ __forceinline__ float rect_min_sigma(float mx, float my, float a, float b, float c,
-                                                float inv_a, float inv_c, const QuadRect& r) {
-  float lx = r.x0 - mx, hx = r.x1 - mx, ly = r.y0 - my, hy = r.y1 - my;
-  if (lx <= 0.f && hx >= 0.f && ly <= 0.f && hy >= 0.f) return 0.f;
-  float s0 = edge_min_sigma(lx, a, c, b, inv_c, ly, hy);
-  float s1 = edge_min_sigma(hx, a, c, b, inv_c, ly, hy);
-  float s2 = edge_min_sigma(ly, c, a, b, inv_a, lx, hx);
-  float s3 = edge_min_sigma(hy, c, a, b, inv_a, lx, hx);
-  return fminf(fminf(s0, s1), fminf(s2, s3));
-}
-
-__device__ __forceinline__ unsigned quadrant_mask(float mx, float my, float a, float b, float c,
-                                                  float opac, float tile_x, float tile_y) {
-  if (!(opac >= kAlphaMin)) return 0u;
-  float thr = 0.6931471805599453f * __builtin_amdgcn_logf(255.0f * opac);
-  float inv_a = __builtin_amdgcn_rcpf(a), inv_c = __builtin_amdgcn_rcpf(c);
-  float fx = fmaxf(fabsf(tile_x - mx), fabsf(tile_x + 16.f - mx));
-  float fy = fmaxf(fabsf(tile_y - my), fabsf(tile_y + 16.f - my));
-  float slack = 0.05f + 4e-6f * (fabsf(a) + fabsf(c) + 2.f * fabsf(b)) * (fx * fx + fy * fy);
-  float lim = thr + slack;
-  unsigned m = 0;
-#pragma unroll
-  for (int k = 0; k < 4; ++k) {
-    QuadRect r;
-    r.x0 = tile_x + 8.f * (k & 1) + 0.5f;
-    r.x1 = r.x0 + 7.f;
-    r.y0 = tile_y + 8.f * (k >> 1) + 0.5f;
-    r.y1 = r.y0 + 7.f;
-    float s = rect_min_sigma(mx, my, a, b, c, inv_a, inv_c, r);
-    if (!(s > lim)) m |= 1u << k;
-  }
-  return m;
-}
 
 __device__ __forceinline__ bool sigma_sign_is_safe(float a, float b, float c) {
   const float tr = a + c;
diff --git a/robosimgs_amd/csrc/tile_cull.h b/robosimgs_amd/csrc/tile_cull.h
--- /dev/null
+++ b/robosimgs_amd/csrc/tile_cull.h
@@ -0,0 +1,96 @@
+#ifndef MGS_TILE_CULL_H_
+#define MGS_TILE_CULL_H_
+
+#include <math.h>
+
+#if defined(__HIPCC__)
+#define MGS_CULL_FN __device__ __forceinline__
+#define MGS_CULL_LOG2(x) __builtin_amdgcn_logf(x)
+#define MGS_CULL_RCP(x) __builtin_amdgcn_rcpf(x)
+#else
+#define MGS_CULL_FN inline
+#define MGS_CULL_LOG2(x) log2f(x)
+#define MGS_CULL_RCP(x) (1.0f / (x))
+#endif
+
+namespace mgs {
+
+constexpr float kAlphaMin = 1.0f / 255.0f;
+
+struct QuadRect { float x0, x1, y0, y1; };
+
+MGS_CULL_FN float edge_min_sigma(float e, float wu, float wv, float b, float inv_wv, float lo, float hi) {
+  float v = fminf(fmaxf(-b * e * inv_wv, lo), hi);
+  return 0.5f * (wu * e * e + wv * v * v) + b * e * v;
+}
+
+MGS_CULL_FN float rect_min_sigma(float mx, float my, float a, float b, float c, float inv_a, float inv_c,
+                                 const QuadRect& r) {
+  float lx = r.x0 - mx, hx = r.x1 - mx, ly = r.y0 - my, hy = r.y1 - my;
+  if (lx <= 0.f && hx >= 0.f && ly <= 0.f && hy >= 0.f) return 0.f;
+  float s0 = edge_min_sigma(lx, a, c, b, inv_c, ly, hy);
+  float s1 = edge_min_sigma(hx, a, c, b, inv_c, ly, hy);
+  float s2 = edge_min_sigma(ly, c, a, b, inv_a, lx, hx);
+  float s3 = edge_min_sigma(hy, c, a, b, inv_a, lx, hx);
+  return fminf(fminf(s0, s1), fminf(s2, s3));
+}
+
+struct CullTerms { float thr, inv_a, inv_c; };
+MGS_CULL_FN CullTerms cull_terms(float a, float c, float opac) {
+  CullTerms t;
+  t.thr = 0.6931471805599453f * MGS_CULL_LOG2(255.0f * opac);
+  t.inv_a = MGS_CULL_RCP(a);
+  t.inv_c = MGS_CULL_RCP(c);
+  return t;
+}
+MGS_CULL_FN float cull_limit(float thr, float mx, float my, float a, float b, float c, float tile_x, float tile_y) {
+  float fx = fmaxf(fabsf(tile_x - mx), fabsf(tile_x + 16.f - mx));
+  float fy = fmaxf(fabsf(tile_y - my), fabsf(tile_y + 16.f - my));
+  float slack = 0.05f + 4e-6f * (fabsf(a) + fabsf(c) + 2.f * fabsf(b)) * (fx * fx + fy * fy);
+  return thr + slack;
+}
+
+MGS_CULL_FN unsigned quadrant_mask(float mx, float my, float a, float b, float c, float opac, float tile_x,
+                                   float tile_y) {
+  if (!(opac >= kAlphaMin)) return 0u;
+  const CullTerms t = cull_terms(a, c, opac);
+  float lim = cull_limit(t.thr, mx, my, a, b, c, tile_x, tile_y);
+  unsigned m = 0;
+#if defined(__HIPCC__)
+#pragma unroll
+#endif
+  for (int k = 0; k < 4; ++k) {
+    QuadRect r;
+    r.x0 = tile_x + 8.f * (k & 1) + 0.5f;
+    r.x1 = r.x0 + 7.f;
+    r.y0 = tile_y + 8.f * (k >> 1) + 0.5f;
+    r.y1 = r.y0 + 7.f;
+    float s = rect_min_sigma(mx, my, a, b, c, t.inv_a, t.inv_c, r);
+    if (!(s > lim)) m |= 1u << k;
+  }
+  return m;
+}
+
+MGS_CULL_FN float rect_min_sigma_facing(float mx, float my, float a, float b, float c, float inv_a, float inv_c,
+                                        const QuadRect& r) {
+  float lx = r.x0 - mx, hx = r.x1 - mx, ly = r.y0 - my, hy = r.y1 - my;
+  const bool in_x = lx <= 0.f && hx >= 0.f, in_y = ly <= 0.f && hy >= 0.f;
+  float sx = edge_min_sigma(lx > 0.f ? lx : hx, a, c, b, inv_c, ly, hy);
+  float sy = edge_min_sigma(ly > 0.f ? ly : hy, c, a, b, inv_a, lx, hx);
+  if (in_x && in_y) return 0.f;
+  return in_x ? sy : (in_y ? sx : fminf(sx, sy));
+}
+
+MGS_CULL_FN bool tile_unreachable(const CullTerms& t, float mx, float my, float a, float b, float c, float tile_x,
+                                  float tile_y) {
+  const float lim = cull_limit(t.thr, mx, my, a, b, c, tile_x, tile_y);
+  QuadRect r;
+  r.x0 = tile_x + 0.5f;
+  r.x1 = r.x0 + 15.f;
+  r.y0 = tile_y + 0.5f;
+  r.y1 = r.y0 + 15.f;
+  return rect_min_sigma_facing(mx, my, a, b, c, t.inv_a, t.inv_c, r) > lim;
+}
+
+}
+#endif
diff --git a/robosimgs_amd/csrc/tile_rect.h b/robosimgs_amd/csrc/tile_rect.h
--- a/robosimgs_amd/csrc/tile_rect.h
+++ b/robosimgs_amd/csrc/tile_rect.h
@@ -2,6 +2,7 @@
 #define MGS_TILE_RECT_H_
 
 #include "mgs_common.h"
+#include "tile_cull.h"
 
 namespace mgs {
 
@@ -53,9 +54,34 @@
   return r;
 }
 
-__device__ __forceinline__ uint2 pack_tile_rect(const TileRect& r) {
+constexpr int kCornerRect = 64;
+__device__ __forceinline__ uint32_t unreachable_corners(const TileRect& r, float mx, float my, float a, float b,
+                                                        float c, float opac, float tile_size) {
+  const int cnt = r.w * r.h;
+  if (cnt <= 0 || cnt > kCornerRect || !(opac >= kAlphaMin)) return 0u;
+  const CullTerms t = cull_terms(a, c, opac);
+  const float xl = (float)r.x0 * tile_size, xr = (float)(r.x0 + r.w - 1) * tile_size;
+  const float yt = (float)r.y0 * tile_size, yb = (float)(r.y0 + r.h - 1) * tile_size;
+  uint32_t m = 0;
+  m |= tile_unreachable(t, mx, my, a, b, c, xl, yt) ? 1u : 0u;
+  m |= r.w == 1 ? (m & 1u) << 1 : (tile_unreachable(t, mx, my, a, b, c, xr, yt) ? 2u : 0u);
+  if (r.h == 1) return m | (m << 2);
+  m |= tile_unreachable(t, mx, my, a, b, c, xl, yb) ? 4u : 0u;
+  m |= r.w == 1 ? (m & 4u) << 1 : (tile_unreachable(t, mx, my, a, b, c, xr, yb) ? 8u : 0u);
+  return m;
+}
+
+constexpr uint32_t kTileCountMask = 0x0fffffffu;
+__device__ __forceinline__ uint2 pack_tile_rect(const TileRect& r, uint32_t corners = 0u) {
   return make_uint2((uint32_t)r.x0 | ((uint32_t)r.y0 << 10) | ((uint32_t)max(r.w, 1) << 20),
-                    (uint32_t)(r.w * r.h));
+                    (uint32_t)(r.w * r.h) | (corners << 28));
+}
+__device__ __forceinline__ uint32_t tile_rect_count(uint32_t word1) { return word1 & kTileCountMask; }
+__device__ __forceinline__ uint32_t tile_rect_corners(uint32_t word1) { return word1 >> 28; }
+__device__ __forceinline__ uint32_t tile_rect_skip_mask(uint32_t w, uint32_t cnt, uint32_t corners) {
+  if (corners == 0u) return 0u;
+  return (corners & 1u) | (((corners >> 1) & 1u) << ((w - 1u) & 31u)) | (((corners >> 2) & 1u) << ((cnt - w) & 31u)) |
+         (((corners >> 3) & 1u) << ((cnt - 1u) & 31u));
 }
 constexpr uint32_t kEmptyTileRect = 1u << 20;
 
diff --git a/robosimgs_amd/ops.py b/robosimgs_amd/ops.py
--- a/robosimgs_amd/ops.py
+++ b/robosimgs_amd/ops.py
@@ -36,6 +36,7 @@
 FRAMES_CAMERA_ORTHO, FRAMES_CAMERA_FISHEYE = 16, 32
 BIN_TIGHT, BIN_RADIUS_OPACITY_AWARE = 1, 2
 BIN_CAMERA_ORTHO, BIN_CAMERA_FISHEYE = 4, 8
+BIN_CORNERS = 16
 RASTER_BWD_RECORDS_ONLY, RASTER_BWD_SPLAT_SLOTS = 1, 2
 PARAMS_RAW = 64
 PARAMS_OPAC_PLAIN = 128
@@ -110,7 +111,7 @@
         ptr(sh_coeffs), ptr(viewmat), ptr(K), width, height, eps2d, near_plane, far_plane,
         radius_clip, ptr(radii_x(radii)), ptr(means2d), ptr(depths), ptr(conics), ptr(opac), stride,
         ptr(feats), ptr(splats),
-        (BIN_TIGHT if bin_seed == "tight" else 0) | (BIN_RADIUS_OPACITY_AWARE if per_axis else 0) | CAMERA_BIN_FLAGS[int(camera)]
+        {"tight": BIN_TIGHT, "corners": BIN_TIGHT | BIN_CORNERS}.get(bin_seed, 0) | (BIN_RADIUS_OPACITY_AWARE if per_axis else 0) | CAMERA_BIN_FLAGS[int(camera)]
         | (PARAMS_RAW if raw else 0) | (PARAMS_OPAC_PLAIN if keep_plain else 0),
         ptr(seed[0]) if seed else None,
         ptr(seed[1]) if seed else None, ptr(radii[1]) if (per_axis and radii is not None) else None, stream_handle()),
```

Result: no change. 4348, median of 2 (-0.6%).
